# gcorso/DiffDock

Hardware: AMD Instinct MI355X
Metric: poses/sec (20 steps x 40 samples, DiffDock-L score model) (higher is better)
Workload: dtype f32

## Files before the change

diffdock_amd/csrc/api.cpp:

```cpp
#include <cstdlib>
#include <cstring>

#include "model.h"

using namespace ddmi;

struct ddmi_model { Model m; };

static thread_local std::string g_err;

template <class F> static int guard(F&& f) {
  try { f(); return DDMI_OK; }
  catch (const Error& e) { g_err = e.what(); return e.code; }
  catch (const std::exception& e) { g_err = e.what(); return DDMI_ERR_ARG; }
}

extern "C" {

const char* ddmi_last_error(void) { return g_err.c_str(); }

int ddmi_create(const ddmi_config* cfg, int device, ddmi_model** out) {
  return guard([&] {
    DDMI_REQUIRE(cfg && out, DDMI_ERR_ARG, "null argument");
    DDMI_REQUIRE(cfg->struct_size == sizeof(ddmi_config), DDMI_ERR_ARG,
                 "ddmi_config.struct_size != sizeof(ddmi_config) of this library: the caller was built against another include/ddmi.h");
    DDMI_CHECK_HIP(hipSetDevice(device));
    auto* h = new ddmi_model();
    h->m.cfg = *cfg;
    h->m.device = device;
    try { build_weight_spec(h->m); } catch (...) { delete h; throw; }
    {
      const ddmi_exec_options& x = h->m.cfg.exec;
      auto in = [&](int v, int hi, const char* name) {
        if (v < 0 || v > hi) { delete h; throw Error(DDMI_ERR_ARG, std::string("ddmi_config.exec.") + name + ": out of range"); }
      };
      if (h->m.cfg.edge_product < 0 || h->m.cfg.edge_product > 1) { delete h; throw Error(DDMI_ERR_ARG, "ddmi_config.edge_product: 0 (f32) or 1 (bf16x4)"); }
      in(x.streams, 1, "streams"); in(x.dense_rows, 2, "dense_rows"); in(x.shared_tiles, 2, "shared_tiles");
      in(x.packed_granules, 1, "packed_granules"); in(x.merged_granule, 1, "merged_granule"); in(x.pre_reduce, 1, "pre_reduce");
      in(x.hidden_mm, 1, "hidden_mm"); in(x.fc1_batch, 1, "fc1_batch"); in(x.tile_split, 8, "tile_split");
      in(x.tile_split_small, 8, "tile_split_small"); in(x.hidden_grid, 1 << 20, "hidden_grid"); in(x.tp_apply, 3, "tp_apply");
      in(x.tile_per_pose, 1, "tile_per_pose"); in(x.layer_overlap, 2, "layer_overlap");
      in(x.grouped, 2, "grouped"); in(x.grouped_split, 8, "grouped_split"); in(x.vn_build, 1, "vn_build"); in(x.node_update, 3, "node_update"); in(x.tile_split_last, 8, "tile_split_last"); in(x.tile_split_rule, 2, "tile_split_rule"); in(x.group_order, 3, "group_order"); in(x.list_caps, 1, "list_caps"); in(x.time_terms, 1, "time_terms");
      h->m.two_streams = x.streams == 0;
      h->m.fused_dense = x.dense_rows == 0 ? 1 : x.dense_rows == 1 ? 0 : 2;
      h->m.fused_shared = x.shared_tiles == 0 ? 1 : x.shared_tiles == 1 ? 0 : 2;
      h->m.fused_pack = x.packed_granules == 0;
      h->m.fused_tri = x.merged_granule == 0;
      h->m.fused_prered = x.pre_reduce == 0;
      h->m.fused_mm = x.hidden_mm == 0;
      h->m.fc1_batch = x.fc1_batch == 0;
      h->m.fused_ysplit = x.tile_split;
      h->m.fused_ysplit_small = x.tile_split_small;
      h->m.eh_grid = x.hidden_grid > 0 ? x.hidden_grid : 2048;
      h->m.tp_form = x.tp_apply == 0 ? -1 : x.tp_apply - 1;
      h->m.tile_per_pose = x.tile_per_pose != 0;
      h->m.layer_overlap = x.layer_overlap;
      h->m.grouped = x.grouped;
      h->m.grouped_split = x.grouped_split;
      h->m.vn_merge = x.vn_build == 0;
      h->m.node_update = x.node_update >= 1;
      h->m.node_update_wpn = x.node_update == 2 ? 1 : x.node_update == 3 ? 4 : 0;
      h->m.fused_ysplit_last = x.tile_split_last;
      h->m.ys_rounds = x.tile_split_rule != 1;
      h->m.ys_rounds_small = x.tile_split_rule == 2;
      h->m.group_order = x.group_order;
      h->m.tight_caps = x.list_caps == 1;
      h->m.time_terms_fused = x.time_terms == 1;
      {
        int cus = 0;
        if (hipDeviceGetAttribute(&cus, hipDeviceAttributeMultiprocessorCount, device) == hipSuccess && cus >= 16) h->m.n_cus = cus;
      }
    }
    DDMI_CHECK_HIP(hipStreamCreateWithFlags(&h->m.side_stream, hipStreamNonBlocking));
    DDMI_CHECK_HIP(hipEventCreate(&h->m.ev_fork));
    DDMI_CHECK_HIP(hipEventCreate(&h->m.ev_join));
    DDMI_CHECK_HIP(hipEventCreate(&h->m.ev_cross));
    DDMI_CHECK_HIP(hipEventCreate(&h->m.ev_terms));
    *out = h;
  });
}

void ddmi_destroy(ddmi_model* h) {
  if (!h) return;
  Model& m = h->m;
  if (m.side_stream) { (void)hipStreamSynchronize(m.side_stream); (void)hipStreamDestroy(m.side_stream); }
  for (hipEvent_t e : {m.ev_fork, m.ev_join, m.ev_cross, m.ev_terms}) if (e) (void)hipEventDestroy(e);
  for (hipEvent_t e : m.ev_pipe) (void)hipEventDestroy(e);
  delete h;
}

int ddmi_num_weights(ddmi_model* h) { return h ? (int)h->m.spec.size() : DDMI_ERR_ARG; }

int ddmi_weight_spec(ddmi_model* h, int i, const char** key, int64_t shape[4], int* ndim) {
  return guard([&] {
    DDMI_REQUIRE(h && i >= 0 && i < (int)h->m.spec.size(), DDMI_ERR_ARG, "bad index");
    *key = h->m.spec[i].first.c_str();
    *ndim = (int)h->m.spec[i].second.size();
    for (int d = 0; d < *ndim; ++d) shape[d] = h->m.spec[i].second[d];
  });
}

int ddmi_set_weight(ddmi_model* h, const char* key, const float* data, const int64_t* shape, int ndim) {
  return guard([&] {
    DDMI_REQUIRE(h && key && shape && ndim >= 1 && ndim <= 4, DDMI_ERR_ARG, "bad argument");
    int64_t numel = 1;
    for (int d = 0; d < ndim; ++d) numel *= shape[d];
    DDMI_REQUIRE(data || numel == 0, DDMI_ERR_ARG, "null data");
    Model& m = h->m;
    bool known = false;
    for (auto& kv : m.spec) if (kv.first == key) {
      known = true;
      DDMI_REQUIRE((int)kv.second.size() == ndim && std::equal(shape, shape + ndim, kv.second.begin()), DDMI_ERR_KEY,
                   std::string("shape mismatch for ") + key);
    }
    DDMI_REQUIRE(known, DDMI_ERR_KEY, std::string("unexpected state_dict key: ") + key);
    HostTensor t;
    t.shape.assign(shape, shape + ndim);
    if (numel) t.data.assign(data, data + numel);
    m.host_w[key] = std::move(t);
    m.committed = false;
  });
}

int ddmi_commit_weights(ddmi_model* h) {
  return guard([&] { DDMI_REQUIRE(h, DDMI_ERR_ARG, "null model"); DDMI_CHECK_HIP(hipSetDevice(h->m.device)); commit_weights(h->m); });
}

int ddmi_set_table(ddmi_model* h, int kind, const double* data, int64_t n) {
  return guard([&] {
    DDMI_REQUIRE(h && data && n > 1 && (kind == 0 || kind == 1), DDMI_ERR_ARG, "bad table");
    DDMI_CHECK_HIP(hipSetDevice(h->m.device));
    std::vector<float> f(data, data + n);
    float* p = h->m.tpool.upload(f);
    if (kind == 0) { h->m.so3_table = p; h->m.so3_n = (int)n; }
    else { h->m.torus_table = p; h->m.torus_n = (int)n; }
  });
}

int ddmi_set_time_frequencies(ddmi_model* h, const float* freq, int64_t n) {
  return guard([&] {
    DDMI_REQUIRE(h && freq && n == h->m.cfg.sigma_embed_dim / 2, DDMI_ERR_ARG, "need sigma_embed_dim/2 frequencies");
    DDMI_REQUIRE(!h->m.committed, DDMI_ERR_STATE, "set frequencies before ddmi_commit_weights");
    h->m.time_freq_host.assign(freq, freq + n);
  });
}

int ddmi_set_complex(ddmi_model* h, const ddmi_complex* c, ddmi_stream s) {
  return guard([&] {
    DDMI_REQUIRE(h && c, DDMI_ERR_ARG, "null argument");
    DDMI_CHECK_HIP(hipSetDevice(h->m.device));
// ... 145 lines not shown
```

diffdock_amd/csrc/complex.cpp:

```cpp
#include <algorithm>
#include <cmath>
#include <numeric>
#include <string>
#include <cstdlib>

#include "model.h"

namespace ddmi {

struct Model::Cx {
  int B = 0, nL = 0, nR = 0, N = 0, Eb = 0, Err = 0, nT = 0;
  int maxNl = 0, maxNr = 0, Ell_cap = 0, Elr_cap = 0, tor_cap = 32, Et = 0, lig_cap = 33;
  bool uniform = false; int Nl_one = 0, R_one = 0;
  std::vector<int> lig_ptr_h, rec_ptr_h;
  int *lig_batch, *rec_batch, *lig_ptr, *rec_ptr, *lig_x;
  int *bond_src, *bond_dst, *bond_grank, *bond_trank, *bg, *bt; float* bond_attr;
  int *tor_u, *tor_v, *tor_batch, *tor_eu, *tor_ev, *rot_u, *rot_v; unsigned char* mask_rotate = nullptr;
  float* rec_pos; int *rr_src, *rr_dst, *rr_batch; float *rr_dist, *rr_nvec, *rr_ew, *rec_edge_base;
  int *rr_goff, *rr_tgt, *rr_tslot, *rr_arow, *rr_toff, *rr_tlist, *rr_gnode;
  int *keep, *cnt_g2, *cnt_t2, *goff2, *toff2, *tslot_tmp, *tgt2, *tslot2, *arow2;
  ReduceGroup *rg_all_crop, *rg_rr_crop;
  float* rec_node_enc;
  float* rec_node_base; int rec_base_dim = 0;
  float *temb, *hidB, *rec_sig, *ligsig, *ll_gvec, *cross_gvec, *center_gvec, *tr_sig, *rot_sig, *cutoff, *rr_rowbias;
  float *ac_in = nullptr, *ac_h0 = nullptr, *ac_h1 = nullptr, *ac_out = nullptr;
  float* rr_sig_old = nullptr;
  float* embsum;
  std::vector<float*> X;
  int *adjrank, *cnt_g, *cnt_t, *goff_ll, *toff_ll, *ll_tgt, *ll_tslot, *ll_featidx, *ll_batch;
  float *ll_dist, *ll_nvec, *ll_ew, *ll_ea;
  int *pairrank, *cnt_l, *cnt_r, *offs_l, *offs_r, *g1_tgt, *g1_tslot, *g3_tgt, *g3_tslot, *pbatch;
  float *pdist, *pnvec, *pew, *cross_ea;
  float *HE, *P, *Q; float* msg[4];
  const float* x_last = nullptr;
  float *HE_b, *P_b, *Q_b, *rowbias_b;
  float *Pg[9] = {}, *Qg[9] = {}, *rbg[9] = {};
  struct VnSet { int vcap = 0; int *cnt = nullptr, *voff = nullptr, *node = nullptr, *e0 = nullptr, *ne = nullptr;
                 float* rows = nullptr;
                 int* tile_hdr = nullptr; unsigned char* live = nullptr;
                 int* nvn_pad = nullptr;
                 const int *built_goff = nullptr, *built_tgt = nullptr, *built_tslot = nullptr, *built_arow = nullptr;
                 const float *built_nvec = nullptr, *built_ew = nullptr; float built_sgn = 0.f; int built_tbase = -1; long epoch = -1; };
  bool prered = false;
  VnSet vn[9];
  int nA = 0, maxNa = 0, Eaa = 0, Ear = 0, Ela_cap = 0;
  int *atom_batch = nullptr, *atom_ptr = nullptr, *atom_x = nullptr;
  float* atom_pos = nullptr;
  struct StaticEdges { int E = 0; int *goff = nullptr, *toff = nullptr, *arow = nullptr, *tgt = nullptr, *tslot = nullptr; };
  StaticEdges se_aa, se_ar, se_ra;
  int *aa_batch = nullptr, *ar_batch = nullptr;
  float *aa_dist = nullptr, *aa_nvec = nullptr, *aa_ew = nullptr, *atom_edge_base = nullptr;
  float *ar_dist = nullptr, *ar_nvec = nullptr, *ar_edge_base = nullptr, *atom_node_base = nullptr;
  int *la_pairrank = nullptr, *la_cnt_l = nullptr, *la_cnt_a = nullptr, *la_offs_l = nullptr, *la_offs_a = nullptr;
  int *la1_tgt = nullptr, *la1_tslot = nullptr, *la3_tgt = nullptr, *la3_tslot = nullptr, *la_pbatch = nullptr;
  float *la_dist = nullptr, *la_nvec = nullptr, *la_ew = nullptr, *la_ea = nullptr, *la_gvec = nullptr;
  float* msg_aa[9] = {};
  ReduceGroup *rg_aa_all = nullptr, *rg_aa_lig = nullptr;
  long epoch = 0;
  float *Hb = nullptr, *Hb_b = nullptr;
  std::vector<float*> rb_l;
  float* Hbg[9] = {};
  float *HD[2] = {nullptr, nullptr}, *HD_b[2] = {nullptr, nullptr};
  ReduceGroup *rg_all, *rg_lig, *rg_ll, *rg_rr;
  float *c_dist, *c_nvec, *c_ea, *c_attr, *c_hid, *c_W, *c_sh, *c_out, *gp;
  int* c_xrow;
  int *t_cnt, *t_atom; float *t_dist, *t_nvec, *t_ew, *t_bond_nvec, *t_ea, *t_attr, *t_hid, *t_W, *t_sh, *t_out, *t_feat;
  float *s_tr, *s_rot, *s_tor, *s_t = nullptr; long long* s_ids = nullptr;
  long long* s_ids_host = nullptr; hipEvent_t s_ids_ev = nullptr;
  ~Cx() { if (s_ids_host) (void)hipHostFree(s_ids_host); if (s_ids_ev) (void)hipEventDestroy(s_ids_ev); }
};

static hipEvent_t get_event(Model& m) {
  if (!m.free_events.empty()) { hipEvent_t e = m.free_events.back(); m.free_events.pop_back(); return e; }
  hipEvent_t e;
  DDMI_CHECK_HIP(hipEventCreate(&e));
  return e;
}
PhaseTimer::PhaseTimer(Model& model, const char* name, hipStream_t stream) : m(model), s(stream) {
  if (!m.timing) return;
  for (size_t i = 0; i < m.phases.size(); ++i) if (m.phases[i].name == name) idx = (int)i;
  if (idx < 0) { m.phases.push_back({name, 0.0, 0}); idx = (int)m.phases.size() - 1; }
  a = get_event(m); b = get_event(m);
  (void)hipEventRecord(a, s);
}
PhaseTimer::~PhaseTimer() {
  if (idx < 0) return;
  (void)hipEventRecord(b, s);
  m.pending.push_back({idx, a, b});
}
void resolve_timings(Model& m) {
  for (auto& p : m.pending) {
    (void)hipEventSynchronize(p.b);
    float ms = 0.f;
    if (hipEventElapsedTime(&ms, p.a, p.b) == hipSuccess) { m.phases[p.phase].ms += ms; m.phases[p.phase].launches++; }
    m.free_events.push_back(p.a); m.free_events.push_back(p.b);
  }
  m.pending.clear();
}

namespace {

typedef Model::Cx Cx;

template <class T> T* dalloc(Model& m, const char* name, std::vector<int64_t> shape, bool zero = false) {
  size_t n = 1;
  for (auto d : shape) n *= (size_t)std::max<int64_t>(d, 0);
  T* p = m.cpool.alloc<T>(n ? n : 1);
  if (zero) DDMI_CHECK_HIP(hipMemset(p, 0, (n ? n : 1) * sizeof(T)));
  if (name) m.debug[name] = DebugEntry{p, shape, !std::is_same<T, float>::value};
  return p;
}
template <class T> T* dup(Model& m, const char* name, const std::vector<T>& v) {
  T* p = m.cpool.upload(v);
  if (name) m.debug[name] = DebugEntry{p, {(int64_t)v.size()}, !std::is_same<T, float>::value};
  return p;
}

void gemm(const float* A, int lda, const float* W, int ldw, const float* bias, float* C, int ldc, int M, int N, int K,
          int act, hipStream_t s, const int* m_dev = nullptr, const float* rowbias = nullptr, const int* ridx = nullptr,
          int ldrb = 0) {
  GemmArgs g;
  g.A = A; g.lda = lda; g.W = W; g.ldw = ldw; g.bias = bias; g.C = C; g.ldc = ldc; g.M = M; g.N = N; g.K = K; g.act = act;
  g.m_dev = m_dev; g.rowbias = rowbias; g.ridx = ridx; g.ldrb = ldrb;
  launch_gemm(g, s);
}

struct RunGroup {
  int gbase, gcount, tbase, tcount;
  const int *goff, *tgt, *tslot, *arow;
  const float* ea; int ea_rows; const int* ea_rows_dev;
  const float* sig; const int* sig_idx;
  const float *nvec, *ew; float sgn;
  float* msg;
  int vn = -1;
  bool load = false;
  bool swap_pq = false;
  const float* rb_ready = nullptr;
  bool static_topo = false;
};

static long tiles_of(const RunGroup& q) {
  const long gn = std::max(1, q.gcount);
  return std::max(1L, gn * (((long)q.ea_rows / gn + 31) / 32) / 16);
}

static bool vn_fresh(const Cx& c, const RunGroup& g) {
  const Cx::VnSet& vs = c.vn[g.vn];
  return vs.built_goff == g.goff && (vs.epoch == c.epoch || (g.static_topo && vs.epoch >= 0)) && vs.built_tgt == g.tgt && vs.built_tslot == g.tslot &&
         vs.built_arow == g.arow && vs.built_nvec == g.nvec && vs.built_ew == g.ew && vs.built_sgn == g.sgn && vs.built_tbase == g.tbase;
}
static void vn_mark_built(Cx& c, const RunGroup& g) {
  Cx::VnSet& vs = c.vn[g.vn];
  vs.built_goff = g.goff; vs.epoch = c.epoch; vs.built_tgt = g.tgt; vs.built_tslot = g.tslot; vs.built_arow = g.arow;
  vs.built_nvec = g.nvec; vs.built_ew = g.ew; vs.built_sgn = g.sgn; vs.built_tbase = g.tbase;
}
static VnRowsArgs vn_rows_args(const Model& m, const RunGroup& g) {
  const Cx::VnSet& vs = m.cx->vn[g.vn];
  VnRowsArgs vr{};
  vr.arow = g.arow; vr.nvec = g.nvec; vr.ew = g.ew; vr.tslot = g.tslot; vr.sgn = g.sgn; vr.sh_lmax = m.cfg.sh_lmax;
  vr.tgt = g.tgt; vr.tbase = g.tbase;
  vr.vcap = vs.vcap; vr.rows = vs.rows; vr.vn_ne = vs.ne;
  return vr;
}
static const char vn_type[9] = {'R', 'R', 'L', 'L', 'A', 'A', 'A', 'L', 'R'};
static void ensure_vn_all(Model& m, const std::vector<RunGroup>& groups, hipStream_t gs) {
  Cx& c = *m.cx;
  VnListsArgs LA;
  VnRowsArgs rows[VN_GROUPS_MAX];
  const RunGroup* prered_g = nullptr;
  for (auto& g : groups) {
    if (vn_fresh(c, g) || g.gcount <= 0) continue;
    DDMI_REQUIRE(LA.n < VN_GROUPS_MAX, DDMI_ERR_CAPACITY, "more edge groups than virtual-node list slots");
    Cx::VnSet& vs = c.vn[g.vn];
    VnListArgs& a = LA.g[LA.n];
    a = VnListArgs{g.goff, g.gcount, vs.voff, vs.node, vs.e0, nullptr, nullptr, 0, nullptr};
    if (vs.nvn_pad) {
      const bool lig = vn_type[g.vn] == 'L', atom = vn_type[g.vn] == 'A';
      a.node_batch = lig ? c.lig_batch : atom ? c.atom_batch : c.rec_batch;
      a.graph_ptr = lig ? c.lig_ptr : atom ? c.atom_ptr : c.rec_ptr;
      a.n_graphs = c.B; a.nvn_pad = vs.nvn_pad;
    }
    rows[LA.n] = vn_rows_args(m, g);
    if (g.vn == 0 && c.prered) {
      prered_g = &g;
      if (m.cfg.sh_lmax <= 1) { rows[LA.n].tile_hdr = vs.tile_hdr; rows[LA.n].live = vs.live; }
    }
    ++LA.n;
    vn_mark_built(c, g);
  }
  if (LA.n == 0) return;
  PhaseTimer t(m, "vn_build", gs);
  launch_vn_build_all(LA, rows, m.cfg.sh_lmax, gs);
  if (prered_g && m.cfg.sh_lmax > 1) {
    Cx::VnSet& vs = c.vn[0];
    launch_vn_tiles(vs.nvn_pad ? vs.nvn_pad : vs.voff + prered_g->gcount, vs.vcap, vs.rows, vs.ne, vs.tile_hdr, vs.live, gs);
  }
}
static void ensure_vn(Model& m, const RunGroup& g, hipStream_t gs) {
  Cx& c = *m.cx;
  Cx::VnSet& vs = c.vn[g.vn];
  if (vn_fresh(c, g)) return;
  PhaseTimer t(m, "vn_build", gs);
  const VnRowsArgs vr = vn_rows_args(m, g);
  VnPoseTiles pp{};
  if (vs.nvn_pad) {
    const bool lig = vn_type[g.vn] == 'L', atom = vn_type[g.vn] == 'A';
    pp.node_batch = lig ? c.lig_batch : atom ? c.atom_batch : c.rec_batch;
    pp.graph_ptr = lig ? c.lig_ptr : atom ? c.atom_ptr : c.rec_ptr;
    pp.n_graphs = c.B; pp.nvn_pad = vs.nvn_pad;
  }
  launch_vn_build(g.goff, g.gcount, vs.cnt, vs.voff, vs.node, vs.e0, vr, gs, vs.nvn_pad ? &pp : nullptr);
  if (g.vn == 0 && c.prered) launch_vn_tiles(vs.nvn_pad ? vs.nvn_pad : vs.voff + g.gcount, vs.vcap, vs.rows, vs.ne, vs.tile_hdr, vs.live, gs);
  vn_mark_built(c, g);
}

struct GroupRoute { bool bf, dense_rows; };
static GroupRoute group_route(const Model& m, const ConvW& L, const RunGroup& g) {
  GroupRoute r;
  r.bf = m.cfg.edge_product == 1 && !L.fgran_generic && L.maxd <= 3 && m.cfg.sh_lmax <= 1;
  r.dense_rows = m.fused_dense == 2 || (m.fused_dense == 1 && (long)g.ea_rows >= 20L * std::max(1, g.gcount));
  return r;
}

static EdgeHiddenArgs hidden_args(Model& m, const ConvW& L, const RunGroup& g, int wg, const float* P, const float* Q, const float* rb,
                                  float* Hb, const GroupRoute& rt) {
  Cx& c = *m.cx;
  Cx::VnSet& vs = c.vn[g.vn];
  EdgeHiddenArgs h{};
  h.nvn = vs.nvn_pad ? vs.nvn_pad : vs.voff + g.gcount;
  h.vcap = vs.vcap; h.vn_node = vs.node; h.vn_e0 = vs.e0; h.goff = g.goff; h.arow = g.arow; h.tgt = g.tgt;
  h.tbase = g.tbase; h.ea = g.ea; h.ns = m.ns; h.W1 = L.W1p[wg]; h.ldw = L.n_edge; h.P = P; h.Q = Q; h.rowbias = rb; h.ridx = g.sig_idx;
  h.H = L.H; h.NG8 = L.HKq / 8; h.Hb = Hb; h.bf = rt.bf ? 1 : 0;
  h.zero_fill = (!L.fgran_generic && rt.dense_rows) ? 1 : 0;
  if (m.cfg.sh_lmax <= 1) { h.vrows = vs.rows; h.vn_ne = vs.ne; }
  h.grid = m.eh_grid;
  return h;
}

static FusedConvArgs fused_args(Model& m, const ConvW& L, const RunGroup& g, size_t gi, int wg, const float* Xin, const float* Hb,
                                const GroupRoute& rt, bool small_layer, int ys_force) {
  Cx& c = *m.cx;
  Cx::VnSet& vs = c.vn[g.vn];
  FusedConvArgs f{};
  f.nvn = vs.nvn_pad ? vs.nvn_pad : vs.voff + g.gcount;
  f.vcap = vs.vcap; f.vn_node = vs.node; f.vrows = vs.rows; f.vn_ne = vs.ne;
  f.X = Xin; f.gbase = g.gbase; f.wpack = L.wpack[wg]; f.KS = L.KS; f.HK = L.HK; f.Hb = Hb; f.NG8 = L.HKq / 8;
  f.sh_lmax = m.cfg.sh_lmax; f.gran = L.fgran; f.cgt = L.cgt;
  f.max_nb = L.max_nb; f.maxd = L.maxd; f.msg = g.msg; f.generic = L.fgran_generic ? 1 : 0;
  f.dense = rt.dense_rows ? 1 : 0;
  f.bf = rt.bf ? 1 : 0;
  f.tile_hdr = (g.vn == 0 && c.prered) ? vs.tile_hdr : nullptr;
  f.shared = (rt.dense_rows && (m.fused_shared == 2 || (m.fused_shared == 1 && g.load && (long)g.ea_rows >= 48L * std::max(1, g.gcount)))) ? 1 : 0;
  f.prof_slot = (int)gi;
  int ys_req = ys_force > 0 ? ys_force : m.fused_ysplit;
  if (ys_req <= 0) {
    auto round_model = [&](long T) {
      int pick = 1;
      double best = 1e30;
      for (int y = 1; y <= std::min(8, L.n_fgran); ++y) {
        const double rounds = std::ceil((double)T * y / (double)m.n_cus);
        const double cost = rounds * ((double)((L.n_fgran + y - 1) / y) + 0.2);
        if (cost < best - 1e-9) { best = cost; pick = y; }
      }
      return pick;
    };
    if (small_layer && m.ys_rounds_small && tiles_of(g) >= 32) ys_req = round_model(tiles_of(g));
    else if (small_layer) ys_req = (int)std::min(8L, std::max(1L, 768 / tiles_of(g)));
    else if (m.ys_rounds && tiles_of(g) >= m.n_cus) {
      ys_req = round_model(tiles_of(g));
    }
    else ys_req = (int)std::min(6L, std::max(1L, 768 / std::max(1L, ((long)g.gcount + g.ea_rows / 32) / 16)));
    const int ys_small = m.fused_ysplit_small;
    if (ys_small > 0 && !small_layer && tiles_of(g) < 256) ys_req = ys_small;
  }
  ys_req = std::max(ys_req, (L.n_fgran + 19) / 20);
  const int ys = std::max(1, std::min(std::min(ys_req, 8), L.n_fgran));
  f.ysplit = ys;
  f.gsplit[0] = 0;
  for (int y = 1; y < ys; ++y) {
    int b = L.n_fgran * y / ys;
    while (b < L.n_fgran && b > 0 && L.fgran_unit[b] == L.fgran_unit[b - 1]) ++b;
    f.gsplit[y] = std::max(b, f.gsplit[y - 1]);
  }
  f.gsplit[ys] = L.n_fgran;
  f.n_units = 0;
  for (int gq = 0; gq < L.n_fgran && f.n_units < 48; ++gq)
    if (gq == 0 || L.fgran_unit[gq] != L.fgran_unit[gq - 1]) f.ustart[f.n_units++] = (short)gq;
  for (int y = 0; y < ys; ++y) {
    f.ufirst[y] = 0; f.ucount[y] = 0;
    for (int u = 0; u < f.n_units; ++u)
      if (f.ustart[u] >= f.gsplit[y] && f.ustart[u] < f.gsplit[y + 1]) { if (f.ucount[y] == 0) f.ufirst[y] = (short)u; ++f.ucount[y]; }
  }
// ... 72 lines not shown
    launch_conv_fused(f, gs);
  }
}

static bool grouped_ok(const Model& m, const ConvW& L, const std::vector<RunGroup>& groups) {
  const Cx& c = *m.cx;
  if (!c.Hbg[0] || groups.size() < 2 || groups.size() > 9 || !c.Pg[0]) return false;
  if (L.TL != 2 || !m.fused_mm || m.ns % 16 != 0 || m.ns > 64 || L.fgran_generic || L.maxd > 3 || m.cfg.sh_lmax > 1 || L.n_fgran <= 0) return false;
  if (m.cfg.edge_product != 0) return false;
  if (m.timing && m.timing_level >= 2) return false;
  for (size_t gi = 0; gi < groups.size(); ++gi)
    if (!L.W1p[std::min<int>((int)gi, L.G - 1)] || groups[gi].vn < 0) return false;
  return true;
}
static void run_groups_grouped(Model& m, const ConvW& L, const std::vector<RunGroup>& groups, const float* Xin, hipStream_t s, bool pq_ready) {
  Cx& c = *m.cx;
  const int ns = m.ns, H = L.H;
  if (!pq_ready) {
    PhaseTimer t(m, "conv_fc1_gemms", s);
    GemmBatch gb;
    auto add = [&](const float* A, int lda, const float* W, const float* bias, float* C, int M) {
      if (gb.n == GEMM_BATCH_MAX) { launch_gemm_batch(gb, s); gb.n = 0; }
      GemmArgs& x = gb.g[gb.n++];
      x = GemmArgs{};
      x.A = A; x.lda = lda; x.W = W; x.ldw = L.n_edge; x.bias = bias; x.C = C; x.ldc = H; x.M = M; x.N = H; x.K = ns;
    };
    for (size_t gi = 0; gi < groups.size(); ++gi) {
      const RunGroup& g = groups[gi];
      const int wg = std::min<int>((int)gi, L.G - 1);
      const float* W1p = L.W1p[wg];
      if (g.sig && !g.rb_ready) add(g.sig, ns, W1p, nullptr, c.rbg[gi], c.B);
      add(Xin + (size_t)g.tbase * XS, XS, W1p + (g.swap_pq ? 2 : 1) * ns, nullptr, c.Pg[gi], g.tcount);
      add(Xin + (size_t)g.gbase * XS, XS, W1p + (g.swap_pq ? 1 : 2) * ns, L.b1p[wg], c.Qg[gi], g.gcount);
    }
    launch_gemm_batch(gb, s);
  }
  ensure_vn_all(m, groups, s);
  long tiles = 0;
  for (auto& g : groups) tiles += tiles_of(g);
  int ys = m.grouped_split;
  if (ys <= 0) ys = (int)std::min(8L, std::max(1L, (long)m.grouped_target / std::max(1L, tiles)));
  std::vector<size_t> order(groups.size());
  std::iota(order.begin(), order.end(), 0);
  std::stable_sort(order.begin(), order.end(), [&](size_t a, size_t b) {
    const GroupRoute ra = group_route(m, L, groups[a]), rb_ = group_route(m, L, groups[b]);
    if (ra.dense_rows != rb_.dense_rows) return ra.dense_rows;
    return tiles_of(groups[a]) > tiles_of(groups[b]);
  });
  for (size_t o0 = 0; o0 < order.size(); o0 += FC_GROUPS_MAX) {
    const size_t n = std::min<size_t>(FC_GROUPS_MAX, order.size() - o0);
    EdgeHiddenGroupedArgs HG;
    FusedGroupedArgs FG;
    HG.n = FG.n = (int)n;
    for (size_t k = 0; k < n; ++k) {
      const size_t gi = order[o0 + k];
      const RunGroup& g = groups[gi];
      const int wg = std::min<int>((int)gi, L.G - 1);
      const GroupRoute rt = group_route(m, L, g);
      HG.g[k] = hidden_args(m, L, g, wg, c.Pg[gi], c.Qg[gi], g.sig ? (g.rb_ready ? g.rb_ready : c.rbg[gi]) : nullptr, c.Hbg[g.vn], rt);
      HG.g[k].grid = std::max(64, (int)((long)m.eh_grid * tiles_of(g) / std::max(1L, tiles)));
      FG.g[k] = fused_args(m, L, g, gi, wg, Xin, c.Hbg[g.vn], rt, false, ys);
    }
    {
      PhaseTimer t(m, "k_edge_hidden", s);
      launch_edge_hidden_mm_grouped(HG, s);
    }
    PhaseTimer t(m, "k_conv_fused", s);
    launch_conv_grouped(FG, s);
  }
}

void run_conv(Model& m, const ConvW& L, const std::vector<RunGroup>& groups, const ReduceGroup* rg_dev, int n_rg,
              const float* Xin, float* Xout, int nbase, int ncount, hipStream_t s, int pq_mode = 0, const ConvW* Lnext = nullptr,
              const std::vector<RunGroup>* gnext = nullptr) {
  Cx& c = *m.cx;
  const int ns = m.ns, H = L.H;
  auto node_update = [&]() {
    if (!Lnext) {
      PhaseTimer t(m, "k_reduce_bn", s);
      launch_reduce_bn(rg_dev, n_rg, nbase, ncount, L.D_in, L.D_out, L.has_bn ? L.bn_mean : nullptr,
                       L.has_bn ? L.bn_scale : nullptr, L.has_bn ? L.bn_bias : nullptr, L.residual ? 1 : 0, Xin, Xout, XS, s);
      return;
    }
    PhaseTimer t(m, "k_reduce_bn", s);
    NodeUpdateArgs a{};
    a.groups = rg_dev; a.n_groups = n_rg; a.nbase = nbase; a.ncount = ncount; a.D_in = L.D_in; a.D_out = L.D_out;
    a.bn_mean = L.has_bn ? L.bn_mean : nullptr; a.bn_scale = L.has_bn ? L.bn_scale : nullptr; a.bn_bias = L.has_bn ? L.bn_bias : nullptr;
    a.residual = L.residual ? 1 : 0; a.X_in = Xin; a.X_out = Xout;
    a.ns = ns; a.H = Lnext->H; a.ldw = Lnext->n_edge; a.wpn = m.node_update_wpn;
    for (size_t gi = 0; gi < gnext->size(); ++gi) {
      const RunGroup& g = (*gnext)[gi];
      const int wg = std::min<int>((int)gi, Lnext->G - 1);
      const float* W1p = Lnext->W1p[wg];
      DDMI_REQUIRE(a.n_terms + 2 <= NU_TERMS_MAX, DDMI_ERR_CAPACITY, "k_node_update: more first-Linear terms than slots");
      a.term[a.n_terms++] = NodeTerm{W1p + (g.swap_pq ? 2 : 1) * ns, nullptr, c.Pg[gi], g.tbase, g.tcount};
      a.term[a.n_terms++] = NodeTerm{W1p + (g.swap_pq ? 1 : 2) * ns, Lnext->b1p[wg], c.Qg[gi], g.gbase, g.gcount};
    }
    launch_node_update(a, s);
  };
  bool forked = false;
  if (m.two_streams && m.side_stream && groups.size() > 1) {
    for (auto& g : groups) forked = forked || (g.gbase == 0 && g.gcount == c.nL && c.nR > 0);
    bool any_main = false;
    for (auto& g : groups) any_main = any_main || !(g.gbase == 0 && g.gcount == c.nL);
    forked = forked && any_main;
  }
  long biggest = 1;
  for (auto& q : groups) biggest = std::max(biggest, tiles_of(q));
  const bool small_layer = biggest < 256;
  if (m.grouped == 2 && grouped_ok(m, L, groups)) {
    run_groups_grouped(m, L, groups, Xin, s, pq_mode == 2);
    node_update();
    return;
  }
  bool mm_all = L.TL == 2 && (pq_mode != 0 || (m.fc1_batch && small_layer)) && m.fused_mm && ns % 16 == 0 && ns <= 64 && groups.size() <= 9 && c.Pg[0];
  for (size_t gi = 0; gi < groups.size(); ++gi) mm_all = mm_all && L.W1p[std::min<int>((int)gi, L.G - 1)];
  DDMI_REQUIRE(pq_mode == 0 || mm_all, DDMI_ERR_STATE, "fused node-update route on a layer without batched first-Linear terms");
  if (mm_all && pq_mode != 2) {
    PhaseTimer t(m, "conv_fc1_gemms", s);
    GemmBatch gb;
    auto add = [&](const float* A, int lda, const float* W, const float* bias, float* C, int M) {
      if (gb.n == GEMM_BATCH_MAX) { launch_gemm_batch(gb, s); gb.n = 0; }
      GemmArgs& x = gb.g[gb.n++];
      x = GemmArgs{};
      x.A = A; x.lda = lda; x.W = W; x.ldw = L.n_edge; x.bias = bias; x.C = C; x.ldc = H; x.M = M; x.N = H; x.K = ns;
    };
    for (size_t gi = 0; gi < groups.size(); ++gi) {
      const RunGroup& g = groups[gi];
      const int wg = std::min<int>((int)gi, L.G - 1);
      const float* W1p = L.W1p[wg];
      if (g.sig && !g.rb_ready) add(g.sig, ns, W1p, nullptr, c.rbg[gi], c.B);
      add(Xin + (size_t)g.tbase * XS, XS, W1p + (g.swap_pq ? 2 : 1) * ns, nullptr, c.Pg[gi], g.tcount);
      add(Xin + (size_t)g.gbase * XS, XS, W1p + (g.swap_pq ? 1 : 2) * ns, L.b1p[wg], c.Qg[gi], g.gcount);
    }
    launch_gemm_batch(gb, s);
  }
  if (m.vn_merge) ensure_vn_all(m, groups, s);
  if (forked) {
    DDMI_CHECK_HIP(hipEventRecord(m.ev_fork, s));
    DDMI_CHECK_HIP(hipStreamWaitEvent(m.side_stream, m.ev_fork, 0));
  }
  std::vector<size_t> issue;
  for (int pass = 0; pass < 2; ++pass) {
    std::vector<size_t> part;
    for (size_t gi = 0; gi < groups.size(); ++gi) {
      const bool side_g = forked && groups[gi].gbase == 0 && groups[gi].gcount == c.nL;
      if (side_g == (pass == 1)) part.push_back(gi);
    }
    if (forked && ((m.group_order >> (pass == 1 ? 0 : 1)) & 1)) std::reverse(part.begin(), part.end());
    issue.insert(issue.end(), part.begin(), part.end());
  }
  if (!forked || m.group_order == 0) { issue.clear(); for (size_t gi = 0; gi < groups.size(); ++gi) issue.push_back(gi); }
  for (size_t ii = 0; ii < issue.size(); ++ii) {
    const size_t gi = issue[ii];
    const RunGroup& g = groups[gi];
    const bool side = forked && g.gbase == 0 && g.gcount == c.nL;
    int ys_last = 0;
    if (m.fused_ysplit_last > 0 && !small_layer) {
      bool last_on_stream = true;
      for (size_t jj = ii + 1; jj < issue.size(); ++jj) {
        const size_t gj = issue[jj];
        const bool side_j = forked && groups[gj].gbase == 0 && groups[gj].gcount == c.nL;
        if (side_j == side) last_on_stream = false;
      }
      if (last_on_stream && tiles_of(g) >= 256) ys_last = m.fused_ysplit_last;
    }
// ... 119 lines not shown
    const int nl = c.lig_ptr_h[b + 1] - c.lig_ptr_h[b], nr = c.rec_ptr_h[b + 1] - c.rec_ptr_h[b];
    DDMI_REQUIRE(nl > 0 && nr > 0, DDMI_ERR_ARG, "graph without ligand or receptor nodes");
    c.maxNl = std::max(c.maxNl, nl); c.maxNr = std::max(c.maxNr, nr);
    c.Elr_cap += nl * nr;
    if (nl != c.lig_ptr_h[1]) c.uniform = false;
    for (int i = c.lig_ptr_h[b]; i < c.lig_ptr_h[b + 1]; ++i) lig_batch[i] = b;
    for (int i = c.rec_ptr_h[b]; i < c.rec_ptr_h[b + 1]; ++i) rec_batch[i] = b;
  }
  c.Ell_cap = c.Eb + c.lig_cap * c.nL;
  std::vector<int> atom_ptr_h, atom_batch, aa_tl, aa_gl, ar_atom, ar_rec, aa_batch_h, ar_batch_h;
  struct HostEdges { std::vector<int> goff, toff, arow, tgt, tslot; };
  auto build_static = [&](const std::vector<int>& tl, const std::vector<int>& gl, int n_t, int n_g, int tgt_base) {
    HostEdges h;
    const int E = (int)tl.size();
    h.goff.assign(n_g + 1, 0); h.toff.assign(n_t + 1, 0);
    for (int k = 0; k < E; ++k) {
      DDMI_REQUIRE(tl[k] >= 0 && tl[k] < n_t && gl[k] >= 0 && gl[k] < n_g, DDMI_ERR_ARG, "atom edge index out of range");
      h.goff[gl[k] + 1]++; h.toff[tl[k] + 1]++;
    }
    for (int i = 0; i < n_g; ++i) h.goff[i + 1] += h.goff[i];
    for (int i = 0; i < n_t; ++i) h.toff[i + 1] += h.toff[i];
    h.arow.resize(E); h.tgt.resize(E); h.tslot.resize(E);
    std::vector<int> cur(h.goff.begin(), h.goff.end() - 1), tcur(h.toff.begin(), h.toff.end() - 1);
    for (int k = 0; k < E; ++k) h.arow[cur[gl[k]]++] = k;
    for (int e = 0; e < E; ++e) { const int k = h.arow[e]; h.tgt[e] = tgt_base + tl[k]; h.tslot[e] = tcur[tl[k]]++; }
    return h;
  };
  HostEdges h_aa, h_ar, h_ra;
  if (cfg.all_atoms) {
    atom_ptr_h.assign(cc.atom_ptr, cc.atom_ptr + c.B + 1);
    DDMI_REQUIRE(atom_ptr_h[0] == 0 && atom_ptr_h[c.B] == c.nA, DDMI_ERR_ARG, "atom_ptr does not span the atom array");
    atom_batch.resize(c.nA);
    for (int b = 0; b < c.B; ++b) {
      const int na = atom_ptr_h[b + 1] - atom_ptr_h[b], nl = c.lig_ptr_h[b + 1] - c.lig_ptr_h[b];
      c.maxNa = std::max(c.maxNa, na);
      c.Ela_cap += nl * na;
      for (int i = atom_ptr_h[b]; i < atom_ptr_h[b + 1]; ++i) atom_batch[i] = b;
    }
    std::vector<int> aa_index(2 * (size_t)c.Eaa), ar_index(2 * (size_t)c.Ear);
    DDMI_CHECK_HIP(hipMemcpy(aa_index.data(), cc.atom_edge_index, aa_index.size() * 4, hipMemcpyDeviceToHost));
    DDMI_CHECK_HIP(hipMemcpy(ar_index.data(), cc.atom_rec_edge_index, ar_index.size() * 4, hipMemcpyDeviceToHost));
    aa_tl.assign(aa_index.begin(), aa_index.begin() + c.Eaa); aa_gl.assign(aa_index.begin() + c.Eaa, aa_index.end());
    ar_atom.assign(ar_index.begin(), ar_index.begin() + c.Ear); ar_rec.assign(ar_index.begin() + c.Ear, ar_index.end());
    h_aa = build_static(aa_tl, aa_gl, c.nA, c.nA, c.nL + c.nR);
    h_ar = build_static(ar_atom, ar_rec, c.nA, c.nR, c.nL + c.nR);
    h_ra = build_static(ar_rec, ar_atom, c.nR, c.nA, c.nL);
    aa_batch_h.resize(c.Eaa); ar_batch_h.resize(c.Ear);
    for (int k = 0; k < c.Eaa; ++k) aa_batch_h[k] = atom_batch[aa_tl[k]];
    for (int k = 0; k < c.Ear; ++k) ar_batch_h[k] = atom_batch[ar_atom[k]];
  }
  std::vector<int> bsrc(c.Eb), bdst(c.Eb), bgr(c.Eb), btr(c.Eb), bg(c.nL, 0), bt(c.nL, 0);
  for (int k = 0; k < c.Eb; ++k) {
    bsrc[k] = bond_index[k]; bdst[k] = bond_index[c.Eb + k];
    DDMI_REQUIRE(bsrc[k] >= 0 && bsrc[k] < c.nL && bdst[k] >= 0 && bdst[k] < c.nL, DDMI_ERR_ARG, "bond index out of range");
    bgr[k] = bg[bdst[k]]++;
    btr[k] = bt[bsrc[k]]++;
  }
  std::vector<int> tor_u, tor_v, tor_b;
  for (int k = 0; k < c.Eb && !cfg.no_torsion; ++k)
    if (edge_mask[k]) { tor_u.push_back(bsrc[k]); tor_v.push_back(bdst[k]); tor_b.push_back(lig_batch[bsrc[k]]); }
  DDMI_REQUIRE((int)tor_u.size() == c.nT, DDMI_ERR_ARG, "n_tor does not equal edge_mask.sum()");
  c.Et = c.nT * c.tor_cap;
  std::vector<int> tor_eu(c.Et), tor_ev(c.Et);
  for (int t = 0; t < c.nT; ++t)
    for (int r = 0; r < c.tor_cap; ++r) { tor_eu[t * c.tor_cap + r] = tor_u[t]; tor_ev[t * c.tor_cap + r] = tor_v[t]; }
  std::vector<int> rr_src(c.Err), rr_dst(c.Err), rr_batch(c.Err), goff(c.nR + 1, 0), toff(c.nR + 1, 0);
  for (int k = 0; k < c.Err; ++k) {
    rr_src[k] = rr_index[k]; rr_dst[k] = rr_index[c.Err + k];
    DDMI_REQUIRE(rr_src[k] >= 0 && rr_src[k] < c.nR && rr_dst[k] >= 0 && rr_dst[k] < c.nR, DDMI_ERR_ARG, "receptor edge out of range");
    rr_batch[k] = rec_batch[rr_src[k]];
    goff[rr_dst[k] + 1]++; toff[rr_src[k] + 1]++;
  }
  for (int i = 0; i < c.nR; ++i) { goff[i + 1] += goff[i]; toff[i + 1] += toff[i]; }
  std::vector<int> rr_arow(c.Err), rr_tgt(c.Err), rr_tslot(c.Err), cur(goff.begin(), goff.end() - 1), tcur(toff.begin(), toff.end() - 1);
  for (int k = 0; k < c.Err; ++k) rr_arow[cur[rr_dst[k]]++] = k;
  std::vector<int> rr_tlist(c.Err), rr_gnode(c.Err);
  for (int e = 0; e < c.Err; ++e) {
    const int k = rr_arow[e];
    rr_tgt[e] = c.nL + rr_src[k];
    rr_tslot[e] = tcur[rr_src[k]]++;
    rr_tlist[rr_tslot[e]] = e;
    rr_gnode[e] = rr_dst[k];
  }
  if (cfg.all_atoms) {
    c.atom_batch = dup(m, "atom_batch", atom_batch); c.atom_ptr = dup(m, nullptr, atom_ptr_h);
    c.atom_x = dalloc<int>(m, nullptr, {c.nA * 4});
    DDMI_CHECK_HIP(hipMemcpy(c.atom_x, cc.atom_x, (size_t)c.nA * 4 * 4, hipMemcpyDeviceToDevice));
    c.atom_pos = dalloc<float>(m, nullptr, {c.nA * 3});
    DDMI_CHECK_HIP(hipMemcpy(c.atom_pos, cc.atom_pos, (size_t)c.nA * 12, hipMemcpyDeviceToDevice));
    auto up_edges = [&](const HostEdges& h, const char* name) {
      Cx::StaticEdges e;
      e.E = (int)h.arow.size();
      e.goff = dup(m, name, h.goff); e.toff = dup(m, nullptr, h.toff); e.arow = dup(m, nullptr, h.arow);
      e.tgt = dup(m, nullptr, h.tgt); e.tslot = dup(m, nullptr, h.tslot);
      return e;
    };
    c.se_aa = up_edges(h_aa, "aa_goff"); c.se_ar = up_edges(h_ar, "ar_goff"); c.se_ra = up_edges(h_ra, "ra_goff");
    c.aa_batch = dup(m, nullptr, aa_batch_h); c.ar_batch = dup(m, nullptr, ar_batch_h);
    int* aa_src = dup(m, nullptr, aa_tl); int* aa_dst = dup(m, nullptr, aa_gl);
    int* ar_src = dup(m, nullptr, ar_atom); int* ar_dst = dup(m, nullptr, ar_rec);
    c.aa_dist = dalloc<float>(m, nullptr, {c.Eaa}); c.aa_nvec = dalloc<float>(m, nullptr, {c.Eaa, 3});
    c.aa_ew = cfg.smooth_edges ? dalloc<float>(m, nullptr, {c.Eaa}) : nullptr;
    c.ar_dist = dalloc<float>(m, nullptr, {c.Ear}); c.ar_nvec = dalloc<float>(m, nullptr, {c.Ear, 3});
    c.atom_edge_base = dalloc<float>(m, nullptr, {c.Eaa, ns}); c.ar_edge_base = dalloc<float>(m, nullptr, {c.Ear, ns});
    c.atom_node_base = dalloc<float>(m, "atom_node_base", {c.nA, XS}, true);
    launch_rec_edge_geom(c.atom_pos, aa_src, aa_dst, c.Eaa, cfg.smooth_edges ? cfg.lig_max_radius : 0.f, c.aa_dist, c.aa_nvec,
                         c.aa_ew, s);
    float* rp = dalloc<float>(m, nullptr, {c.nR * 3});
    DDMI_CHECK_HIP(hipMemcpy(rp, cc.rec_pos, (size_t)c.nR * 12, hipMemcpyDeviceToDevice));
    launch_rec_edge_geom(c.atom_pos, ar_src, ar_dst, c.Ear, 0.f, c.ar_dist, c.ar_nvec, nullptr, s, rp);
  }
  c.lig_batch = dup(m, "lig_batch", lig_batch); c.rec_batch = dup(m, "rec_batch", rec_batch);
  c.lig_ptr = dup(m, nullptr, c.lig_ptr_h); c.rec_ptr = dup(m, nullptr, c.rec_ptr_h);
  c.lig_x = dalloc<int>(m, nullptr, {c.nL * 16});
  DDMI_CHECK_HIP(hipMemcpy(c.lig_x, cc.lig_x, (size_t)c.nL * 16 * 4, hipMemcpyDeviceToDevice));
  c.bond_src = dup(m, nullptr, bsrc); c.bond_dst = dup(m, nullptr, bdst); c.bond_grank = dup(m, nullptr, bgr);
  c.bond_trank = dup(m, nullptr, btr); c.bg = dup(m, nullptr, bg); c.bt = dup(m, nullptr, bt);
  c.bond_attr = dalloc<float>(m, nullptr, {c.Eb * m.nf});
  if (c.Eb) DDMI_CHECK_HIP(hipMemcpy(c.bond_attr, cc.bond_attr, (size_t)c.Eb * m.nf * 4, hipMemcpyDeviceToDevice));
  c.tor_u = dup(m, "tor_u", tor_u); c.tor_v = dup(m, "tor_v", tor_v); c.tor_batch = dup(m, nullptr, tor_b);
  c.tor_eu = dup(m, nullptr, tor_eu); c.tor_ev = dup(m, nullptr, tor_ev);
  if (c.uniform && c.nT % c.B == 0) {
    c.Nl_one = c.nL / c.B; c.R_one = c.nT / c.B;
    std::vector<int> ru(tor_u.begin(), tor_u.begin() + c.R_one), rv(tor_v.begin(), tor_v.begin() + c.R_one);
    c.rot_u = dup(m, nullptr, ru); c.rot_v = dup(m, nullptr, rv);
    if (cc.mask_rotate && c.R_one > 0) {
      c.mask_rotate = dalloc<unsigned char>(m, nullptr, {c.R_one * c.Nl_one});
      DDMI_CHECK_HIP(hipMemcpy(c.mask_rotate, cc.mask_rotate, (size_t)c.R_one * c.Nl_one, hipMemcpyDeviceToDevice));
    }
  }
  c.rec_pos = dalloc<float>(m, nullptr, {c.nR * 3});
  DDMI_CHECK_HIP(hipMemcpy(c.rec_pos, cc.rec_pos, (size_t)c.nR * 12, hipMemcpyDeviceToDevice));
  c.rr_src = dup(m, nullptr, rr_src); c.rr_dst = dup(m, nullptr, rr_dst); c.rr_batch = dup(m, nullptr, rr_batch);
  c.rr_goff = dup(m, "rr_goff", goff); c.rr_toff = dup(m, "rr_toff", toff); c.rr_arow = dup(m, nullptr, rr_arow);
  c.rr_tgt = dup(m, nullptr, rr_tgt); c.rr_tslot = dup(m, nullptr, rr_tslot);
  c.rr_tlist = dup(m, nullptr, rr_tlist); c.rr_gnode = dup(m, nullptr, rr_gnode);
  c.keep = dalloc<int>(m, "crop_keep", {c.nR}); c.cnt_g2 = dalloc<int>(m, nullptr, {c.nR}); c.cnt_t2 = dalloc<int>(m, nullptr, {c.nR});
  c.goff2 = dalloc<int>(m, "rr_goff_crop", {c.nR + 1}); c.toff2 = dalloc<int>(m, nullptr, {c.nR + 1});
  c.tslot_tmp = dalloc<int>(m, nullptr, {c.Err}); c.tgt2 = dalloc<int>(m, nullptr, {c.Err});
  c.tslot2 = dalloc<int>(m, nullptr, {c.Err}); c.arow2 = dalloc<int>(m, nullptr, {c.Err});
  const int B = c.B, nL = c.nL, nR = c.nR, N = c.N;
  c.rr_dist = dalloc<float>(m, nullptr, {c.Err}); c.rr_nvec = dalloc<float>(m, nullptr, {c.Err, 3});
  c.rr_ew = cfg.smooth_edges ? dalloc<float>(m, nullptr, {c.Err}) : nullptr;
  c.rec_edge_base = dalloc<float>(m, "rec_edge_base", {c.Err, ns});
  c.rec_node_base = dalloc<float>(m, "rec_node_base", {nR, XS}, true);
  c.temb = dalloc<float>(m, "temb", {B, sd}); c.hidB = dalloc<float>(m, nullptr, {B, std::max(ns, H)});
  c.rec_sig = dalloc<float>(m, "rec_sig", {B, ns}); c.ligsig = dalloc<float>(m, nullptr, {B, ns});
  c.ll_gvec = dalloc<float>(m, nullptr, {B, ns}); c.cross_gvec = dalloc<float>(m, nullptr, {B, ns});
  c.center_gvec = dalloc<float>(m, nullptr, {B, ns}); c.tr_sig = dalloc<float>(m, nullptr, {B, ns});
  c.rr_sig_old = dalloc<float>(m, nullptr, {B, ns});
  if (cfg.atom_confidence && cfg.confidence_mode) {
    c.ac_in = dalloc<float>(m, nullptr, {nL, 2 * ns}); c.ac_h0 = dalloc<float>(m, nullptr, {nL, ns});
    c.ac_h1 = dalloc<float>(m, nullptr, {nL, ns}); c.ac_out = dalloc<float>(m, nullptr, {nL, cfg.atom_num_confidence_outputs + ns});
  }
  c.rot_sig = dalloc<float>(m, nullptr, {B, ns}); c.cutoff = dalloc<float>(m, "cross_cutoff", {B});
  c.rr_rowbias = dalloc<float>(m, nullptr, {B, H});
  c.embsum = dalloc<float>(m, nullptr, {nL, ns});
  const int n_layers = cfg.old_model ? cfg.num_conv_layers + 2 : (int)m.conv_layers.size(), K = (int)m.lig_emb_layers.size();
  for (int l = 0; l <= n_layers + K; ++l) {
    static const char* names[] = {"x0", "x1", "x2", "x3", "x4", "x5", "x6", "x7", "x8", "x9", "x10", "x11", "x12"};
    c.X.push_back(dalloc<float>(m, l < 13 ? names[l] : nullptr, {N, XS}, true));
  }
  c.adjrank = dalloc<int>(m, nullptr, {nL, c.maxNl}); c.cnt_g = dalloc<int>(m, nullptr, {nL}); c.cnt_t = dalloc<int>(m, nullptr, {nL});
  c.goff_ll = dalloc<int>(m, "goff_ll", {nL + 1}); c.toff_ll = dalloc<int>(m, "toff_ll", {nL + 1});
  c.ll_tgt = dalloc<int>(m, "ll_tgt", {c.Ell_cap}); c.ll_tslot = dalloc<int>(m, nullptr, {c.Ell_cap});
  c.ll_featidx = dalloc<int>(m, nullptr, {c.Ell_cap}); c.ll_batch = dalloc<int>(m, nullptr, {c.Ell_cap});
  c.ll_dist = dalloc<float>(m, "ll_dist", {c.Ell_cap}); c.ll_nvec = dalloc<float>(m, nullptr, {c.Ell_cap, 3});
  c.ll_ew = cfg.smooth_edges ? dalloc<float>(m, nullptr, {c.Ell_cap}) : nullptr;
  c.ll_ea = dalloc<float>(m, "ll_ea", {c.Ell_cap, ns});
  c.pairrank = dalloc<int>(m, nullptr, {nL, c.maxNr}); c.cnt_l = dalloc<int>(m, nullptr, {nL}); c.cnt_r = dalloc<int>(m, nullptr, {nR});
  c.offs_l = dalloc<int>(m, "offs_l", {nL + 1}); c.offs_r = dalloc<int>(m, "offs_r", {nR + 1});
  c.g1_tgt = dalloc<int>(m, nullptr, {c.Elr_cap}); c.g1_tslot = dalloc<int>(m, nullptr, {c.Elr_cap});
  c.g3_tgt = dalloc<int>(m, nullptr, {c.Elr_cap}); c.g3_tslot = dalloc<int>(m, nullptr, {c.Elr_cap});
  c.pbatch = dalloc<int>(m, nullptr, {c.Elr_cap}); c.pdist = dalloc<float>(m, "cross_dist", {c.Elr_cap});
  c.pnvec = dalloc<float>(m, nullptr, {c.Elr_cap, 3}); c.pew = cfg.smooth_edges ? dalloc<float>(m, nullptr, {c.Elr_cap}) : nullptr;
  c.cross_ea = dalloc<float>(m, "cross_ea", {c.Elr_cap, ns});
  const int max_rows = std::max(std::max(std::max(c.Ell_cap, c.Elr_cap), std::max(c.Err, c.Eaa)), std::max(c.Ear, c.Ela_cap));
  c.HE = dalloc<float>(m, nullptr, {max_rows, H}); c.P = dalloc<float>(m, nullptr, {N, H}); c.Q = dalloc<float>(m, nullptr, {N, H});
  c.HE_b = dalloc<float>(m, nullptr, {std::max(std::max(c.Ell_cap, c.Elr_cap), c.Ela_cap), H}); c.P_b = dalloc<float>(m, nullptr, {N, H});
  c.Q_b = dalloc<float>(m, nullptr, {N, H}); c.rowbias_b = dalloc<float>(m, nullptr, {B, H});
  if (cfg.tp_weights_layers > 2) {
    for (int i = 0; i < 2; ++i) {
      c.HD[i] = dalloc<float>(m, nullptr, {max_rows, H});
      c.HD_b[i] = dalloc<float>(m, nullptr, {std::max(std::max(c.Ell_cap, c.Elr_cap), c.Ela_cap), H});
    }
  }
  for (int i = 0; i < (cfg.all_atoms ? 9 : 4); ++i) {
    c.Pg[i] = dalloc<float>(m, nullptr, {N, H}); c.Qg[i] = dalloc<float>(m, nullptr, {N, H}); c.rbg[i] = dalloc<float>(m, nullptr, {B, H});
  }
  for (size_t l = 0; l < m.conv_layers.size(); ++l) c.rb_l.push_back(dalloc<float>(m, nullptr, {B, H}));
  std::vector<const ConvW*> all_layers;
  for (auto* fam : {&m.conv_layers, &m.lig_emb_layers, &m.rec_emb_layers, &m.old_lig, &m.old_rec, &m.old_l2r, &m.old_r2l})
    for (auto& L : *fam) all_layers.push_back(&L);
  {
    int HKq = 0;
    for (auto* L : all_layers) HKq = std::max(HKq, L->HKq);
    const int ecap_v[9] = {c.Elr_cap, c.Err, c.Ell_cap, c.Elr_cap, c.Ela_cap, c.Ear, c.Eaa, c.Ela_cap, c.Ear};
    const int gn_v[9] = {nR, nR, nL, nL, c.nA, c.nA, c.nA, nL, nR};
    const bool lig_v[9] = {false, false, true, true, false, false, false, true, false};
    const char* names[9] = {"vn_off_cross", "vn_off_rr", "vn_off_ll", "vn_off_rl", "vn_off_la", "vn_off_ra", "vn_off_aa",
                            "vn_off_al", "vn_off_ar"};
    long tight[9];
    for (int i = 0; i < 9; ++i) tight[i] = -1;
    auto vn_of = [](long deg) { return (deg + 31) / 32; };
    auto exact = [&](const std::vector<int>& off) { long n = 0; for (size_t d = 0; d + 1 < off.size(); ++d) n += vn_of(off[d + 1] - off[d]); return n; };
    tight[0] = tight[3] = 0;
    for (int b = 0; b < B; ++b) {
      const long nl = c.lig_ptr_h[b + 1] - c.lig_ptr_h[b], nr = c.rec_ptr_h[b + 1] - c.rec_ptr_h[b];
      tight[0] += nr * vn_of(nl);
      tight[3] += nl * vn_of(nr);
    }
    tight[1] = exact(goff);
    tight[2] = 0;
    for (int d = 0; d < nL; ++d) tight[2] += vn_of((long)c.lig_cap + bg[d]);
    if (cfg.all_atoms) {
      tight[4] = tight[7] = 0;
      for (int b = 0; b < B; ++b) {
        const long nl = c.lig_ptr_h[b + 1] - c.lig_ptr_h[b], na = atom_ptr_h[b + 1] - atom_ptr_h[b];
        tight[4] += na * vn_of(nl);
        tight[7] += nl * vn_of(na);
      }
      tight[5] = exact(h_ra.goff); tight[6] = exact(h_aa.goff); tight[8] = exact(h_ar.goff);
    }
    int vmax = 0, vmax_b = 0;
    for (int i = 0; i < (cfg.all_atoms ? 9 : 4); ++i) {
      Cx::VnSet& vs = c.vn[i];
      vs.vcap = gn_v[i] + ecap_v[i] / 32 + 2;
      if (m.tight_caps && tight[i] >= 0) vs.vcap = (int)std::min<long>(vs.vcap, tight[i] + 2);
      if (m.tile_per_pose) {
        vs.vcap += 16 * B;
        vs.nvn_pad = dalloc<int>(m, i == 0 ? "vn_count_cross" : nullptr, {1}, true);
      }
      vs.cnt = dalloc<int>(m, nullptr, {gn_v[i] + 1}); vs.voff = dalloc<int>(m, names[i], {gn_v[i] + 1});
      vs.node = dalloc<int>(m, nullptr, {vs.vcap}); vs.e0 = dalloc<int>(m, nullptr, {vs.vcap});
      const int shd = (cfg.sh_lmax + 1) * (cfg.sh_lmax + 1);
      vs.ne = dalloc<int>(m, i == 0 ? "vn_ne_cross" : nullptr, {round_up(vs.vcap, 16)});
      vs.rows = dalloc<float>(m, nullptr, {round_up(vs.vcap, 16), 32, shd == 4 ? 8 : shd + 3});
      if (i == 0) {
        c.prered = m.fused_prered && shd == 4 && !cfg.old_model && !m.conv_layers.empty() && m.fused_shared != 2;
        for (auto& L : m.conv_layers) c.prered = c.prered && !L.fgran_generic && L.maxd <= 3 && L.n_fgran > 0;
        if (c.prered) {
          vs.tile_hdr = dalloc<int>(m, "prered_tile_hdr", {round_up(vs.vcap, 16) / 16, FC_TILE_HDR}, true);
          vs.live = dalloc<unsigned char>(m, nullptr, {ecap_v[0]}, true);
        }
      }
      vmax = std::max(vmax, vs.vcap);
      if (lig_v[i]) vmax_b = std::max(vmax_b, vs.vcap);
    }
    c.Hb = HKq > 0 ? dalloc<float>(m, nullptr, {round_up(vmax, 16), 32, round_up(HKq, 16)}) : nullptr;
    if (m.grouped == 2 && HKq > 0)
      for (int i = 0; i < (cfg.all_atoms ? 9 : 4); ++i) c.Hbg[i] = dalloc<float>(m, nullptr, {round_up(c.vn[i].vcap, 16), 32, round_up(HKq, 16)});
    c.Hb_b = HKq > 0 ? dalloc<float>(m, nullptr, {round_up(vmax_b, 16), 32, round_up(HKq, 16)}) : nullptr;
  }
  const int ecap[4] = {c.Ell_cap, c.Elr_cap, c.Err, c.Elr_cap};
  for (int g = 0; g < 4; ++g) c.msg[g] = dalloc<float>(m, nullptr, {ecap[g], XS});
  {
    std::vector<ReduceGroup> rg = {{c.toff_ll, c.msg[0], 0, nL}, {c.offs_l, c.msg[1], 0, nL},
                                   {c.rr_toff, c.msg[2], nL, nR}, {c.offs_r, c.msg[3], nL, nR}};
    rg[1].live = c.prered ? c.vn[0].live : nullptr;
    c.rg_all = m.cpool.upload(rg);
    std::vector<ReduceGroup> rl(rg.begin(), rg.begin() + 2);
    c.rg_lig = m.cpool.upload(rl);
    std::vector<ReduceGroup> r0(rg.begin(), rg.begin() + 1);
    c.rg_ll = m.cpool.upload(r0);
    std::vector<ReduceGroup> r2 = {{c.rr_toff, c.msg[2], 0, nR}};
    c.rg_rr = m.cpool.upload(r2);
    std::vector<ReduceGroup> rc = rg;
    rc[2].toff = c.toff2;
    c.rg_all_crop = m.cpool.upload(rc);
    std::vector<ReduceGroup> r2c = {{c.toff2, c.msg[2], nL, nR}};
    c.rg_rr_crop = m.cpool.upload(r2c);
    if (cfg.all_atoms) {
      const int nA = c.nA;
      c.la_pairrank = dalloc<int>(m, nullptr, {nL, c.maxNa}); c.la_cnt_l = dalloc<int>(m, nullptr, {nL});
      c.la_cnt_a = dalloc<int>(m, nullptr, {nA}); c.la_offs_l = dalloc<int>(m, "offs_la_l", {nL + 1});
      c.la_offs_a = dalloc<int>(m, "offs_la_a", {nA + 1});
      c.la1_tgt = dalloc<int>(m, nullptr, {c.Ela_cap}); c.la1_tslot = dalloc<int>(m, nullptr, {c.Ela_cap});
      c.la3_tgt = dalloc<int>(m, nullptr, {c.Ela_cap}); c.la3_tslot = dalloc<int>(m, nullptr, {c.Ela_cap});
      c.la_pbatch = dalloc<int>(m, nullptr, {c.Ela_cap}); c.la_dist = dalloc<float>(m, nullptr, {c.Ela_cap});
      c.la_nvec = dalloc<float>(m, nullptr, {c.Ela_cap, 3});
      c.la_ew = cfg.smooth_edges ? dalloc<float>(m, nullptr, {c.Ela_cap}) : nullptr;
      c.la_ea = dalloc<float>(m, nullptr, {c.Ela_cap, ns}); c.la_gvec = dalloc<float>(m, nullptr, {B, ns});
      const int ecap9[9] = {c.Ell_cap, c.Elr_cap, c.Ela_cap, c.Err, c.Elr_cap, c.Ear, c.Eaa, c.Ela_cap, c.Ear};
      for (int g = 0; g < 9; ++g) c.msg_aa[g] = (g == 0 || g == 1 || g == 3 || g == 4) ? c.msg[g == 0 ? 0 : g == 1 ? 1 : g == 3 ? 2 : 3]
                                                                                          : dalloc<float>(m, nullptr, {ecap9[g], XS});
      std::vector<ReduceGroup> r9 = {{c.toff_ll, c.msg_aa[0], 0, nL}, {c.offs_l, c.msg_aa[1], 0, nL}, {c.la_offs_l, c.msg_aa[2], 0, nL},
                                     {c.rr_toff, c.msg_aa[3], nL, nR}, {c.offs_r, c.msg_aa[4], nL, nR}, {c.se_ra.toff, c.msg_aa[5], nL, nR},
                                     {c.se_aa.toff, c.msg_aa[6], nL + nR, nA}, {c.la_offs_a, c.msg_aa[7], nL + nR, nA},
                                     {c.se_ar.toff, c.msg_aa[8], nL + nR, nA}};
      r9[1].live = c.prered ? c.vn[0].live : nullptr;
      c.rg_aa_all = m.cpool.upload(r9);
      std::vector<ReduceGroup> r3(r9.begin(), r9.begin() + 3);
      c.rg_aa_lig = m.cpool.upload(r3);
    }
  }
  const ConvW& F = m.final_conv;
  c.c_dist = dalloc<float>(m, nullptr, {nL}); c.c_nvec = dalloc<float>(m, nullptr, {nL, 3});
  c.c_ea = dalloc<float>(m, nullptr, {nL, ns}); c.c_attr = dalloc<float>(m, nullptr, {nL, F.n_edge});
  c.c_hid = dalloc<float>(m, nullptr, {nL, F.H}); c.c_W = dalloc<float>(m, nullptr, {nL, F.Wn});
  c.c_sh = dalloc<float>(m, nullptr, {nL, F.sh_dim}); c.c_out = dalloc<float>(m, nullptr, {nL, F.D_out});
  c.gp = dalloc<float>(m, "global_pred", {B, F.D_out});
  {
    std::vector<int> xr(nL);
    std::iota(xr.begin(), xr.end(), 0);
    c.c_xrow = m.cpool.upload(xr);
  }
  if (c.nT > 0) {
    const ConvW& T = m.tor_conv;
    c.t_cnt = dalloc<int>(m, "tor_cnt", {c.nT}); c.t_atom = dalloc<int>(m, nullptr, {c.Et});
    c.t_dist = dalloc<float>(m, nullptr, {c.Et}); c.t_nvec = dalloc<float>(m, nullptr, {c.Et, 3});
    c.t_ew = cfg.smooth_edges ? dalloc<float>(m, nullptr, {c.Et}) : nullptr;
    c.t_bond_nvec = dalloc<float>(m, nullptr, {c.nT, 3}); c.t_ea = dalloc<float>(m, nullptr, {c.Et, ns});
    c.t_attr = dalloc<float>(m, nullptr, {c.Et, T.n_edge}); c.t_hid = dalloc<float>(m, nullptr, {c.Et, T.H});
    c.t_W = dalloc<float>(m, nullptr, {c.Et, T.Wn}); c.t_sh = dalloc<float>(m, nullptr, {c.Et, T.sh_dim});
    c.t_out = dalloc<float>(m, nullptr, {c.Et, T.D_out}); c.t_feat = dalloc<float>(m, "tor_feat", {c.nT, T.D_out});
  }
  c.s_tr = dalloc<float>(m, nullptr, {B, 3}); c.s_rot = dalloc<float>(m, nullptr, {B, 3});
  c.s_tor = dalloc<float>(m, nullptr, {std::max(c.nT, 1)});
  c.s_t = nullptr; c.s_ids = nullptr;

  launch_rec_edge_geom(c.rec_pos, c.rr_src, c.rr_dst, c.Err, cfg.smooth_edges ? cfg.rec_max_radius : 0.f, c.rr_dist, c.rr_nvec,
                       c.rr_ew, s);
  if (!cfg.old_model)
    launch_edge_mlp(mlp_args(m.rec_edge, ns, c.Err, nullptr, c.rr_dist, m.off_rec, m.D, m.coeff_rec, 0, m.rec_edge.b0, nullptr,
                             c.rec_edge_base), s);
  if (cfg.old_model) {
    std::vector<int> ident(nR);
    std::iota(ident.begin(), ident.end(), 0);
    int* rid = m.cpool.upload(ident);
    float* cat = dalloc<float>(m, nullptr, {nR, ns + m.lm});
    launch_concat_rec_input(cc.rec_x, 1 + m.lm, m.rec_emb, ns, m.lm, nR, cat, s);
    if (m.lm > 0) {
      float* emb1 = dalloc<float>(m, nullptr, {nR, ns});
      gemm(cat + ns, ns + m.lm, m.old_rec_lin.W0, sd, m.old_rec_lin.b0, emb1, ns, nR, ns, sd, 0, s, nullptr, cat, rid, ns + m.lm);
      gemm(emb1, ns, m.old_lm_W, ns + m.lm, m.old_lm_b, c.rec_node_base, XS, nR, ns, ns, 0, s);
      gemm(cat + ns + sd, ns + m.lm, m.old_lm_W + ns, ns + m.lm, nullptr, c.rec_node_base, XS, nR, ns, m.lm - sd, 0, s, nullptr,
           c.rec_node_base, rid, XS);
    } else {
      launch_add_rowvec(c.rec_node_base, XS, cat, ns, nullptr, 0, nullptr, nR, ns, 0, s);
    }
  } else if (m.lm > 0) {
    float* cat = dalloc<float>(m, nullptr, {nR, ns + m.lm});
    launch_concat_rec_input(cc.rec_x, 1 + m.lm, m.rec_emb, ns, m.lm, nR, cat, s);
    gemm(cat, ns + m.lm, m.rec_enc_W, ns + m.lm, m.rec_enc_b, c.rec_node_base, XS, nR, ns, ns + m.lm, 0, s);
  } else {
    float* cat = dalloc<float>(m, nullptr, {nR, ns});
    launch_concat_rec_input(cc.rec_x, 1, m.rec_emb, ns, 0, nR, cat, s);
    launch_add_rowvec(c.rec_node_base, XS, cat, ns, nullptr, 0, nullptr, nR, ns, 0, s);
  }
  c.rec_base_dim = ns;
  if (cfg.all_atoms) {
    float* emb = dalloc<float>(m, nullptr, {c.nA, ns});
    launch_lig_node_embed(c.atom_x, c.nA, m.atom_emb, m.atom_emb_off, 4, ns, emb, s);
    launch_add_rowvec(c.atom_node_base, XS, emb, ns, nullptr, 0, nullptr, c.nA, ns, 0, s);
    launch_edge_mlp(mlp_args(m.atom_edge, ns, c.Eaa, nullptr, c.aa_dist, m.off_lig, m.D, m.coeff_lig, 0, m.atom_edge.b0, nullptr,
                             c.atom_edge_base), s);
    launch_edge_mlp(mlp_args(m.ar_edge, ns, c.Ear, nullptr, c.ar_dist, m.off_rec, m.D, m.coeff_rec, 0, m.ar_edge.b0, nullptr,
                             c.ar_edge_base), s);
  }
  c.rec_node_enc = nullptr;
  if (!m.rec_emb_layers.empty() && cfg.all_atoms) {
    const int aB = nL + nR, nA = c.nA;
    float* ea = dalloc<float>(m, nullptr, {N, XS}, true);
    float* eb = dalloc<float>(m, nullptr, {N, XS}, true);
    DDMI_CHECK_HIP(hipMemcpyAsync(ea + (size_t)nL * XS, c.rec_node_base, (size_t)nR * XS * 4, hipMemcpyDeviceToDevice, s));
    DDMI_CHECK_HIP(hipMemcpyAsync(ea + (size_t)aB * XS, c.atom_node_base, (size_t)nA * XS * 4, hipMemcpyDeviceToDevice, s));
    RunGroup e_rr{nL, nR, nL, nR, c.rr_goff, c.rr_tgt, c.rr_tslot, c.rr_arow, c.rec_edge_base, c.Err, nullptr, nullptr, nullptr,
                  c.rr_nvec, c.rr_ew, 1.f, c.msg_aa[3]};
    RunGroup e_ar{nL, nR, aB, nA, c.se_ar.goff, c.se_ar.tgt, c.se_ar.tslot, c.se_ar.arow, c.ar_edge_base, c.Ear, nullptr, nullptr,
                  nullptr, c.ar_nvec, nullptr, 1.f, c.msg_aa[8]};
    RunGroup e_aa{aB, nA, aB, nA, c.se_aa.goff, c.se_aa.tgt, c.se_aa.tslot, c.se_aa.arow, c.atom_edge_base, c.Eaa, nullptr, nullptr,
                  nullptr, c.aa_nvec, c.aa_ew, 1.f, c.msg_aa[6]};
    RunGroup e_ra{aB, nA, nL, nR, c.se_ra.goff, c.se_ra.tgt, c.se_ra.tslot, c.se_ra.arow, c.ar_edge_base, c.Ear, nullptr, nullptr,
                  nullptr, c.ar_nvec, nullptr, 1.f, c.msg_aa[5]};
    e_rr.vn = 1; e_ar.vn = 8; e_aa.vn = 6; e_ra.vn = 5;
    std::vector<ReduceGroup> re = {{c.rr_toff, c.msg_aa[3], nL, nR}, {c.se_ar.toff, c.msg_aa[8], aB, nA},
                                   {c.se_aa.toff, c.msg_aa[6], aB, nA}, {c.se_ra.toff, c.msg_aa[5], nL, nR}};
    ReduceGroup* rg_emb = m.cpool.upload(re);
    float *xin = ea, *xout = eb;
    for (size_t i = 0; i < m.rec_emb_layers.size(); ++i) {
      run_conv(m, m.rec_emb_layers[i], {e_rr, e_ar, e_aa, e_ra}, rg_emb, 4, xin, xout, nL, nR + nA, s);
      std::swap(xin, xout);
      c.rec_base_dim = m.rec_emb_layers[i].D_out;
    }
    DDMI_CHECK_HIP(hipMemcpyAsync(c.rec_node_base, xin + (size_t)nL * XS, (size_t)nR * XS * 4, hipMemcpyDeviceToDevice, s));
    DDMI_CHECK_HIP(hipMemcpyAsync(c.atom_node_base, xin + (size_t)aB * XS, (size_t)nA * XS * 4, hipMemcpyDeviceToDevice, s));
  } else if (!m.rec_emb_layers.empty()) {
    c.rec_node_enc = dalloc<float>(m, nullptr, {nR, XS}, true);
    DDMI_CHECK_HIP(hipMemcpyAsync(c.rec_node_enc, c.rec_node_base, (size_t)nR * XS * 4, hipMemcpyDeviceToDevice, s));
    std::vector<int> tgt_local(c.Err);
    for (int e = 0; e < c.Err; ++e) tgt_local[e] = rr_tgt[e] - c.nL;
    int* tl = m.cpool.upload(tgt_local);
    float* xa = dalloc<float>(m, nullptr, {nR, XS}, true);
    float* xin = c.rec_node_base;
    for (size_t i = 0; i < m.rec_emb_layers.size(); ++i) {
      const ConvW& L = m.rec_emb_layers[i];
      RunGroup g{0, nR, 0, nR, c.rr_goff, tl, c.rr_tslot, c.rr_arow, c.rec_edge_base, c.Err, nullptr, nullptr, nullptr,
                 c.rr_nvec, c.rr_ew, 1.f, c.msg[2]};
      g.vn = 1;
      float* xout = (xin == c.rec_node_base) ? xa : c.rec_node_base;
      run_conv(m, L, {g}, c.rg_rr, 1, xin, xout, 0, nR, s);
      xin = xout;
      c.rec_base_dim = L.D_out;
    }
    if (xin != c.rec_node_base)
      DDMI_CHECK_HIP(hipMemcpyAsync(c.rec_node_base, xin, (size_t)nR * XS * 4, hipMemcpyDeviceToDevice, s));
  }
  DDMI_CHECK_HIP(hipStreamSynchronize(s));
  m.has_complex = true;
}

static void score_readouts(Model& m, const float* XL, const float* lig_pos, const float* t_tr, const float* t_rot,
                           const float* t_tor, float* tr_out, float* rot_out, float* tor_out, hipStream_t s) {
  Cx& c = *m.cx;
  const ddmi_config& cfg = m.cfg;
  const int ns = m.ns, sd = m.sd, B = c.B, nL = c.nL;
  if (m.two_streams && m.side_stream && c.nT > 0 && tor_out) {
    DDMI_CHECK_HIP(hipEventRecord(m.ev_fork, s));
    DDMI_CHECK_HIP(hipStreamWaitEvent(m.side_stream, m.ev_fork, 0));
  }
  const ConvW& F = m.final_conv;
  launch_center_prep(lig_pos, c.lig_batch, c.lig_ptr, nL, cfg.sh_lmax, XL, cfg.fixed_center_conv ? c.c_xrow : c.lig_batch, ns, c.c_dist,
                     c.c_nvec, c.c_sh, F.sh_dim, c.c_attr, F.n_edge, s);
  {
    EdgeMlpArgs ea = mlp_args(m.center_edge, ns, nL, nullptr, c.c_dist, m.off_center, m.D, m.coeff_center, 0, c.center_gvec, c.lig_batch, c.c_attr);
    ea.ldo = F.n_edge;
    launch_edge_mlp(ea, s);
  }
  run_direct_conv(m, F, c.c_attr, nL, c.c_hid, c.c_W, c.c_xrow, XL, c.c_sh, nullptr, nullptr, 0, c.c_out, s);
  launch_segment_mean_bn(c.c_out, F.D_out, c.lig_ptr, nullptr, 0, B, F.D_out, F.has_bn ? F.bn_mean : nullptr,
                         F.has_bn ? F.bn_scale : nullptr, F.has_bn ? F.bn_bias : nullptr, c.gp, F.D_out, s);
  {
    ScoreHeadArgs a{};
    a.B = B; a.gp = c.gp; a.odd_parity = cfg.odd_parity; a.scale_by_sigma = cfg.scale_by_sigma; a.ns = ns; a.ldw0 = 1 + sd;
    a.tr_w0n = m.tr_final.W0; a.tr_sig = c.tr_sig; a.tr_w3 = m.tr_final.W3; a.tr_b3 = m.tr_final.b3;
    a.rot_w0n = m.rot_final.W0; a.rot_sig = c.rot_sig; a.rot_w3 = m.rot_final.W3; a.rot_b3 = m.rot_final.b3;
    a.t_tr = t_tr; a.t_rot = t_rot; a.tr_smin = cfg.tr_sigma_min; a.tr_smax = cfg.tr_sigma_max;
    a.rot_smin = cfg.rot_sigma_min; a.rot_smax = cfg.rot_sigma_max; a.so3_table = m.so3_table; a.so3_n = m.so3_n;
    a.tr_out = tr_out; a.rot_out = rot_out;
    launch_score_heads(a, s);
  }
  if (c.nT > 0 && tor_out) {
    const ConvW& T = m.tor_conv;
    const hipStream_t s_main = s;
    const bool fork = m.two_streams && m.side_stream;
    if (fork) s = m.side_stream;
    launch_tor_radius(lig_pos, c.lig_ptr, c.tor_u, c.tor_v, c.tor_batch, c.nT, cfg.lig_max_radius, c.tor_cap,
                      cfg.smooth_edges ? cfg.lig_max_radius : 0.f, c.t_cnt, c.t_atom, c.t_dist, c.t_nvec, c.t_ew, c.t_bond_nvec, s);
    {
      EdgeMlpArgs ea = mlp_args(m.final_edge, ns, c.Et, nullptr, c.t_dist, m.off_lig, m.D, m.coeff_lig, 0, m.final_edge.b0, nullptr, c.t_attr);
      ea.ldo = T.n_edge;
      launch_edge_mlp(ea, s);
    }
    launch_tor_prep(c.t_nvec, c.t_bond_nvec, c.nT, c.tor_cap, cfg.sh_lmax, m.tor_T, m.tor_ds, m.tor_dts, c.t_sh, XL, c.t_atom, c.tor_eu,
                    c.tor_ev, ns, c.t_attr, T.n_edge, s);
    run_direct_conv(m, T, c.t_attr, c.Et, c.t_hid, c.t_W, c.t_atom, XL, c.t_sh, c.t_ew, c.t_cnt, c.tor_cap, c.t_out, s);
    launch_segment_mean_bn(c.t_out, T.D_out, nullptr, c.t_cnt, c.tor_cap, c.nT, T.D_out, T.has_bn ? T.bn_mean : nullptr,
                           T.has_bn ? T.bn_scale : nullptr, T.has_bn ? T.bn_bias : nullptr, c.t_feat, T.D_out, s);
    TorHeadArgs a{};
    a.nT = c.nT; a.ns = ns; a.in_dim = T.D_out; a.feat = c.t_feat; a.W0 = m.tor_W0; a.W3 = m.tor_W3;
    a.tor_batch = c.tor_batch; a.t_tor = t_tor; a.smin = cfg.tor_sigma_min; a.smax = cfg.tor_sigma_max;
    a.scale_by_sigma = cfg.scale_by_sigma; a.torus_table = m.torus_table; a.torus_n = m.torus_n; a.out = tor_out;
    launch_tor_head(a, s);
    if (fork) {
      DDMI_CHECK_HIP(hipEventRecord(m.ev_join, m.side_stream));
      DDMI_CHECK_HIP(hipStreamWaitEvent(s_main, m.ev_join, 0));
    }
  }
}

static void forward_old(Model& m, const float* lig_pos, const float* t_tr, const float* t_rot, const float* t_tor, float* tr_out,
                        float* rot_out, float* tor_out, float* conf_out, hipStream_t s) {
  Cx& c = *m.cx;
  const ddmi_config& cfg = m.cfg;
  const int ns = m.ns, sd = m.sd, B = c.B, nL = c.nL, nR = c.nR, Lc = cfg.num_conv_layers;
  ++c.epoch;
  PhaseTimer t_fwd(m, "forward_total", s);
  std::unique_ptr<PhaseTimer> t_phase(new PhaseTimer(m, "embed_and_graphs", s));
  launch_time_embedding(t_tr, B, m.time_freq, sd / 2, cfg.embedding_scale, cfg.embedding_type, c.temb, s);
  gemm(c.temb, sd, m.old_lig_lin.W0, sd, m.old_lig_lin.b0, c.ligsig, ns, B, ns, sd, 0, s);
  if (m.lm > 0) gemm(c.temb, sd, m.old_lm_W + ns + m.lm - sd, ns + m.lm, nullptr, c.rec_sig, ns, B, ns, sd, 0, s);
  else gemm(c.temb, sd, m.old_rec_lin.W0, sd, m.old_rec_lin.b0, c.rec_sig, ns, B, ns, sd, 0, s);
  gemm(c.temb, sd, m.lig_edge.W0 + m.nf, m.lig_edge.in, m.lig_edge.b0, c.ll_gvec, ns, B, ns, sd, 0, s);
  gemm(c.temb, sd, m.cross_edge.W0, m.cross_edge.in, m.cross_edge.b0, c.cross_gvec, ns, B, ns, sd, 0, s);
  gemm(c.temb, sd, m.rec_edge.W0, m.rec_edge.in, m.rec_edge.b0, c.rr_sig_old, ns, B, ns, sd, 0, s);
  const bool conf = cfg.confidence_mode != 0;
  if (!conf) {
    gemm(c.temb, sd, m.center_edge.W0 + m.D, m.center_edge.in, m.center_edge.b0, c.center_gvec, ns, B, ns, sd, 0, s);
    gemm(c.temb, sd, m.tr_final.W0 + 1, 1 + sd, m.tr_final.b0, c.tr_sig, ns, B, ns, sd, 0, s);
    gemm(c.temb, sd, m.rot_final.W0 + 1, 1 + sd, m.rot_final.b0, c.rot_sig, ns, B, ns, sd, 0, s);
  }
// ... 191 lines not shown
  if (crop && !m.rec_emb_layers.empty()) {
    launch_add_rowvec(c.X[0] + (size_t)nL * XS, XS, c.rec_node_enc, XS, nullptr, 0, nullptr, nR, ns, 0, s);
    RunGroup g_rr0{nL, nR, nL, nR, c.goff2, c.tgt2, c.tslot2, c.arow2, c.rec_edge_base, c.Err, nullptr, nullptr,
                   nullptr, c.rr_nvec, c.rr_ew, 1.f, c.msg[2]};
    g_rr0.vn = 1;
    for (size_t i = 0; i < m.rec_emb_layers.size(); ++i)
      run_conv(m, m.rec_emb_layers[i], {g_rr0}, c.rg_rr_crop, 1, c.X[i], c.X[i + 1], nL, nR, s);
    launch_add_rowvec(c.X[xi] + (size_t)nL * XS, XS, c.X[xi] + (size_t)nL * XS, XS, c.rec_sig, ns, c.rec_batch, nR,
                      c.rec_base_dim, ns, s);
  } else if (!nodes_on_side) {
    launch_add_rowvec(c.X[xi] + (size_t)nL * XS, XS, c.rec_node_base, XS, c.rec_sig, ns, c.rec_batch, nR, c.rec_base_dim, ns, s);
  }
  if (early_cross) DDMI_CHECK_HIP(hipStreamWaitEvent(s, m.ev_cross, 0));
  else cross_graph(s, keep);
  RunGroup g_lr{nL, nR, 0, nL, c.offs_r, c.g1_tgt, c.g1_tslot, c.g1_tslot, c.cross_ea, c.Elr_cap, c.offs_l + nL, nullptr,
                      nullptr, c.pnvec, c.pew, 1.f, c.msg[1]};
  RunGroup g_rr{nL, nR, nL, nR, crop ? c.goff2 : c.rr_goff, crop ? c.tgt2 : c.rr_tgt, crop ? c.tslot2 : c.rr_tslot,
                      crop ? c.arow2 : c.rr_arow, c.rec_edge_base, c.Err, nullptr, c.rec_sig, c.rr_batch, c.rr_nvec, c.rr_ew,
                      1.f, c.msg[2]};
  RunGroup g_rl{0, nL, nL, nR, c.offs_l, c.g3_tgt, c.g3_tslot, nullptr, c.cross_ea, c.Elr_cap, c.offs_l + nL, nullptr,
                nullptr, c.pnvec, c.pew, -1.f, c.msg[3]};
  g_lr.vn = 0; g_rr.vn = 1; g_rl.vn = 3; g_rl.load = true;
  g_rr.static_topo = !crop;
  const int Lc = (int)m.conv_layers.size();
  if (cfg.all_atoms) {
    const int nA = c.nA, aB = nL + nR;
    launch_add_rowvec(c.X[xi] + (size_t)aB * XS, XS, c.atom_node_base, XS, c.rec_sig, ns, c.atom_batch, nA, c.rec_base_dim, ns, s);
    launch_cross_count(lig_pos, c.atom_pos, c.lig_batch, c.atom_batch, c.lig_ptr, c.atom_ptr, nL, nA, c.maxNa, nullptr,
                       cfg.lig_max_radius, nullptr, c.la_pairrank, c.la_cnt_l, c.la_cnt_a, s);
    launch_exclusive_scan2(c.la_cnt_l, c.la_offs_l, nL, c.la_cnt_a, c.la_offs_a, nA, s);
    launch_cross_fill(lig_pos, c.atom_pos, c.atom_batch, c.lig_ptr, c.atom_ptr, nL, nA, c.maxNa, c.la_pairrank, c.la_offs_l,
                      c.la_offs_a, nullptr, cfg.lig_max_radius, cfg.smooth_edges, c.la1_tgt, c.la1_tslot, c.la3_tgt, c.la3_tslot,
                      c.la_pbatch, c.la_dist, c.la_nvec, c.la_ew, s, aB);
    gemm(c.temb, sd, m.la_edge.W0, m.la_edge.in, m.la_edge.b0, c.la_gvec, ns, B, ns, sd, 0, s);
    launch_edge_mlp(mlp_args(m.la_edge, ns, c.Ela_cap, c.la_offs_l + nL, c.la_dist, m.off_lig, m.D, m.coeff_lig, sd, c.la_gvec,
                             c.la_pbatch, c.la_ea), s);
    RunGroup a_ll = g_ll, a_lr = g_lr, a_rr = g_rr, a_rl = g_rl;
    a_rl.sgn = 1.f;
    a_ll.msg = c.msg_aa[0]; a_lr.msg = c.msg_aa[1]; a_rr.msg = c.msg_aa[3]; a_rl.msg = c.msg_aa[4];
    RunGroup a_la{aB, nA, 0, nL, c.la_offs_a, c.la1_tgt, c.la1_tslot, c.la1_tslot, c.la_ea, c.Ela_cap, c.la_offs_l + nL, nullptr,
                  nullptr, c.la_nvec, c.la_ew, 1.f, c.msg_aa[2]};
    RunGroup a_ra{aB, nA, nL, nR, c.se_ra.goff, c.se_ra.tgt, c.se_ra.tslot, c.se_ra.arow, c.ar_edge_base, c.Ear, nullptr, c.rec_sig,
                  c.ar_batch, c.ar_nvec, nullptr, 1.f, c.msg_aa[5]};
    RunGroup a_aa{aB, nA, aB, nA, c.se_aa.goff, c.se_aa.tgt, c.se_aa.tslot, c.se_aa.arow, c.atom_edge_base, c.Eaa, nullptr, c.rec_sig,
                  c.aa_batch, c.aa_nvec, c.aa_ew, 1.f, c.msg_aa[6]};
    RunGroup a_al{0, nL, aB, nA, c.la_offs_l, c.la3_tgt, c.la3_tslot, nullptr, c.la_ea, c.Ela_cap, c.la_offs_l + nL, nullptr,
                  nullptr, c.la_nvec, c.la_ew, 1.f, c.msg_aa[7]};
    RunGroup a_ar{nL, nR, aB, nA, c.se_ar.goff, c.se_ar.tgt, c.se_ar.tslot, c.se_ar.arow, c.ar_edge_base, c.Ear, nullptr, c.rec_sig,
                  c.ar_batch, c.ar_nvec, nullptr, 1.f, c.msg_aa[8]};
    a_la.vn = 4; a_ra.vn = 5; a_aa.vn = 6; a_al.vn = 7; a_al.load = true; a_ar.vn = 8;
    a_ra.static_topo = a_aa.static_topo = a_ar.static_topo = true;
    t_phase.reset();
    for (int l = 0; l < Lc; ++l, ++xi) {
      if (l < Lc - 1)
        run_conv(m, m.conv_layers[l], {a_ll, a_lr, a_la, a_rr, a_rl, a_ra, a_aa, a_al, a_ar}, c.rg_aa_all, 9, c.X[xi], c.X[xi + 1], 0,
                 c.N, s);
      else run_conv(m, m.conv_layers[l], {a_ll, a_lr, a_la}, c.rg_aa_lig, 3, c.X[xi], c.X[xi + 1], 0, nL, s);
    }
  } else {
    t_phase.reset();
    bool overlapped = m.layer_overlap && m.two_streams && m.side_stream && nR > 0 && Lc >= 2;
    if (overlapped) {
      long biggest = 1;
      for (const RunGroup* q : {&g_ll, &g_lr, &g_rr, &g_rl}) biggest = std::max(biggest, tiles_of(*q));
      overlapped = biggest >= 256 || m.layer_overlap == 2;
    }
    bool nu = m.node_update && !overlapped && Lc >= 2 && m.fused_mm && ns % 16 == 0 && ns <= 64 && c.Pg[0] && (int)c.rb_l.size() == Lc;
    for (auto& L : m.conv_layers) {
      nu = nu && L.TL == 2 && L.H == m.conv_layers[0].H && L.n_edge == m.conv_layers[0].n_edge;
      for (int g = 0; g < 4; ++g) nu = nu && L.W1p[std::min(g, L.G - 1)];
    }
    if (nu) {
      PhaseTimer t(m, "conv_fc1_gemms", s);
      GemmBatch gb;
      for (int l = 0; l < Lc - 1; ++l) {
        const ConvW& L = m.conv_layers[l];
        if (gb.n == GEMM_BATCH_MAX) { launch_gemm_batch(gb, s); gb.n = 0; }
        GemmArgs& x = gb.g[gb.n++];
        x = GemmArgs{};
        x.A = c.rec_sig; x.lda = ns; x.W = L.W1p[std::min(2, L.G - 1)]; x.ldw = L.n_edge; x.C = c.rb_l[l]; x.ldc = L.H; x.M = B; x.N = L.H; x.K = ns;
      }
      if (gb.n) launch_gemm_batch(gb, s);
    }
    if (overlapped) run_conv_layers_overlapped(m, g_ll, g_lr, g_rr, g_rl, crop ? c.rg_all_crop : c.rg_all, xi, s);
    else
    for (int l = 0; l < Lc; ++l, ++xi) {
      RunGroup rr = g_rr;
      if (nu && l < Lc - 1) rr.rb_ready = c.rb_l[l];
      const std::vector<RunGroup> full = {g_ll, g_lr, rr, g_rl}, ligs = {g_ll, g_lr};
      std::vector<RunGroup> next;
      if (nu && l + 1 < Lc) {
        if (l + 1 < Lc - 1) next = {g_ll, g_lr, g_rr, g_rl}; else next = ligs;
      }
      const int pq = !nu ? 0 : l == 0 ? 1 : 2;
      const ConvW* Ln = next.empty() ? nullptr : &m.conv_layers[l + 1];
      if (l < Lc - 1)
        run_conv(m, m.conv_layers[l], full, crop ? c.rg_all_crop : c.rg_all, 4, c.X[xi], c.X[xi + 1], 0, c.N, s, pq, Ln, Ln ? &next : nullptr);
      else run_conv(m, m.conv_layers[l], ligs, c.rg_lig, 2, c.X[xi], c.X[xi + 1], 0, cfg.sidechain_pred ? c.N : nL, s, pq);
    }
  }
  const float* XL = c.X[xi];
  c.x_last = conf ? nullptr : XL;
  PhaseTimer t_read(m, "readouts", s);
  if (conf) {
    const int total = cfg.num_conv_layers + cfg.num_prot_emb_layers;
    const ConvW& Ll = m.conv_layers.back();
    ConfHeadArgs a{};
    a.B = B; a.X = XL; a.ldx = XS; a.col0 = 0; a.lig_ptr = c.lig_ptr; a.ns = ns;
    a.n_tail = total >= 3 ? (cfg.reduce_pseudoscalars ? cfg.nv : ns) : 0;
    a.tail_off = Ll.D_out - a.n_tail;
    if (cfg.atom_confidence) {
      const int n_in = ns + a.n_tail, na = cfg.atom_num_confidence_outputs, wo = na + ns;
      launch_gather_cols(c.ac_in, n_in, 0, XL, XS, nullptr, nL, ns, nullptr, s);
      if (a.n_tail > 0) launch_gather_cols(c.ac_in, n_in, ns, XL + a.tail_off, XS, nullptr, nL, a.n_tail, nullptr, s);
      gemm(c.ac_in, n_in, m.aconf_W[0], n_in, m.aconf_b[0], c.ac_h0, ns, nL, ns, n_in, 1, s);
      gemm(c.ac_h0, ns, m.aconf_W[1], ns, m.aconf_b[1], c.ac_h1, ns, nL, ns, ns, 1, s);
      gemm(c.ac_h1, ns, m.aconf_W[2], ns, m.aconf_b[2], c.ac_out, wo, nL, wo, ns, 0, s);
      launch_gather_cols(atom_conf_out, na, 0, c.ac_out, wo, nullptr, nL, na, nullptr, s);
      a.X = c.ac_out; a.ldx = wo; a.col0 = na; a.n_tail = 0; a.tail_off = 0;
    }
    a.W0 = m.conf_W[0]; a.b0 = m.conf_b[0]; a.sc0 = m.conf_bn_scale[0]; a.sh0 = m.conf_bn_shift[0];
    a.W1 = m.conf_W[1]; a.b1 = m.conf_b[1]; a.sc1 = m.conf_bn_scale[1]; a.sh1 = m.conf_bn_shift[1];
    a.W2 = m.conf_W[2]; a.b2 = m.conf_b[2]; a.n_out = cfg.num_confidence_outputs + (cfg.affinity_prediction ? 1 : 0); a.out = conf_out;
    launch_conf_head(a, s);
    return;
  }
  score_readouts(m, XL, lig_pos, t_tr, t_rot, t_tor, tr_out, rot_out, tor_out, s);
}

void sidechain_pred(Model& m, float* out, hipStream_t s) {
  DDMI_REQUIRE(m.has_complex && m.cx->x_last && m.side_Mt, DDMI_ERR_STATE,
               "ddmi_sidechain_pred reads the node table of the ddmi_forward directly before it (none since the last ddmi_confidence / ddmi_sample / ddmi_set_complex)");
  Cx& c = *m.cx;
  gemm(c.x_last + (size_t)c.nL * XS, XS, m.side_Mt, m.side_K, nullptr, out, 10, c.nR, 10, m.side_K, 0, s);
}

void modify_conformer(Model& m, float* lig_pos, const float* tr, const float* rot, const float* tor, hipStream_t s) {
  DDMI_REQUIRE(m.has_complex, DDMI_ERR_STATE, "ddmi_set_complex must precede ddmi_modify_conformer");
  Cx& c = *m.cx;
  DDMI_REQUIRE(c.uniform && c.Nl_one > 0, DDMI_ERR_STATE,
               "modify_conformer needs a batch of copies of one complex (utils/diffusion_utils.py:60-64)");
  const bool torsion = tor != nullptr && c.R_one > 0;
  DDMI_REQUIRE(!torsion || c.mask_rotate, DDMI_ERR_STATE, "mask_rotate was not provided to ddmi_set_complex");
  launch_modify_conformer(lig_pos, c.B, c.Nl_one, torsion ? c.R_one : 0, c.rot_u, c.rot_v, c.mask_rotate, tr, rot,
                          torsion ? tor : nullptr, s);
}

static const long long* upload_sample_ids(Model& m, const int64_t* ids, hipStream_t s) {
  Cx& c = *m.cx;
  if (!ids) return nullptr;
  if (!c.s_ids) {
    c.s_ids = m.cpool.alloc<long long>(c.B);
    DDMI_CHECK_HIP(hipHostMalloc(reinterpret_cast<void**>(&c.s_ids_host), (size_t)c.B * 8));
    DDMI_CHECK_HIP(hipEventCreate(&c.s_ids_ev));
  } else {
    DDMI_CHECK_HIP(hipEventSynchronize(c.s_ids_ev));
  }
  for (int b = 0; b < c.B; ++b) c.s_ids_host[b] = ids[b];
  DDMI_CHECK_HIP(hipMemcpyAsync(c.s_ids, c.s_ids_host, (size_t)c.B * 8, hipMemcpyHostToDevice, s));
  DDMI_CHECK_HIP(hipEventRecord(c.s_ids_ev, s));
  return c.s_ids;
}

static void perturb_step(Model& m, float* tr, float* rot, float* tor, const ddmi_sample_cfg& sc, int k,
                         const long long* ids_dev, hipStream_t s) {
  Cx& c = *m.cx;
  const ddmi_config& cfg = m.cfg;
  const int steps = sc.inference_steps, B = c.B;
  const bool torsion = tor != nullptr && !cfg.no_torsion && c.nT > 0;
  const bool last = k == steps - 1;
  const double t_tr = sc.tr_schedule[k], t_rot = sc.rot_schedule[k], t_tor = sc.tor_schedule[k];
  const double dt_tr = last ? t_tr : t_tr - sc.tr_schedule[k + 1];
  const double dt_rot = last ? t_rot : t_rot - sc.rot_schedule[k + 1];
  const double dt_tor = last ? t_tor : t_tor - sc.tor_schedule[k + 1];
  const double s_tr = std::pow((double)cfg.tr_sigma_min, 1 - t_tr) * std::pow((double)cfg.tr_sigma_max, t_tr);
  const double s_rot = std::pow((double)cfg.rot_sigma_min, 1 - t_rot) * std::pow((double)cfg.rot_sigma_max, t_rot);
  const double s_tor = std::pow((double)cfg.tor_sigma_min, 1 - t_tor) * std::pow((double)cfg.tor_sigma_max, t_tor);
  const bool zero_noise = sc.no_random || (sc.no_final_step_noise && last) || sc.ode;
  auto coeffs = [&](double sigma, double smin, double smax, double dt, int i, float& cs, float& cz) {
    const double g = sigma * std::sqrt(2.0 * std::log(smax / smin));
    double a = sc.ode ? 0.5 * g * g * dt : g * g * dt;
    double z = g * std::sqrt(dt);
    if (sc.temp_sampling[i] != 1.0) {
      const double T = sc.temp_sampling[i], psi = sc.temp_psi[i], sdat = sc.temp_sigma_data[i];
      const double sigma_data = std::exp(sdat * std::log(smax) + (1 - sdat) * std::log(smin));
      const double lambda = (sigma_data + sigma) / (sigma_data + sigma / T);
      a = g * g * dt * (lambda + T * psi / 2);
      z = g * std::sqrt(dt * (1 + psi));
    }
    cs = (float)a;
    cz = zero_noise ? 0.f : (float)z;
  };
  PerturbArgs p{};
  p.B = B; p.R = torsion ? c.nT / B : 0; p.tr = tr; p.rot = rot; p.tor = tor;
  coeffs(s_tr, cfg.tr_sigma_min, cfg.tr_sigma_max, dt_tr, 0, p.c_tr_s, p.c_tr_z);
  coeffs(s_rot, cfg.rot_sigma_min, cfg.rot_sigma_max, dt_rot, 1, p.c_rot_s, p.c_rot_z);
  coeffs(s_tor, cfg.tor_sigma_min, cfg.tor_sigma_max, dt_tor, 2, p.c_tor_s, p.c_tor_z);
  if (!zero_noise) {
    p.z_tr = sc.z_tr ? sc.z_tr + (size_t)k * B * 3 : nullptr;
    p.z_rot = sc.z_rot ? sc.z_rot + (size_t)k * B * 3 : nullptr;
    p.z_tor = sc.z_tor ? sc.z_tor + (size_t)k * c.nT : nullptr;
    p.use_rng = 1;
  }
  p.seed = sc.seed; p.sample_ids = ids_dev; p.step = k;
  launch_perturb(p, s);
}

static void check_sample_cfg(Model& m, const ddmi_sample_cfg& sc) {
  DDMI_REQUIRE(sc.inference_steps > 0 && sc.tr_schedule && sc.rot_schedule && sc.tor_schedule, DDMI_ERR_ARG, "bad schedule");
  DDMI_REQUIRE(m.cx->uniform, DDMI_ERR_STATE, "the step loop needs a batch of copies of one complex");
}

void perturb(Model& m, float* tr, float* rot, float* tor, const ddmi_sample_cfg& sc, int k, hipStream_t s) {
  DDMI_REQUIRE(m.has_complex, DDMI_ERR_STATE, "ddmi_set_complex must precede ddmi_perturb");
  check_sample_cfg(m, sc);
  DDMI_REQUIRE(k >= 0 && k < sc.inference_steps, DDMI_ERR_ARG, "step index out of range");
  perturb_step(m, tr, rot, tor, sc, k, upload_sample_ids(m, sc.sample_ids, s), s);
}

void sample(Model& m, float* lig_pos, const ddmi_sample_cfg& sc, hipStream_t s) {
  DDMI_REQUIRE(m.has_complex, DDMI_ERR_STATE, "ddmi_set_complex must precede ddmi_sample");
  check_sample_cfg(m, sc);
  Cx& c = *m.cx;
  const ddmi_config& cfg = m.cfg;
  const int steps = sc.inference_steps, B = c.B;
  const bool torsion = !cfg.no_torsion && c.nT > 0;
  struct CropGuard {
    Model& m; double saved;
    ~CropGuard() { m.crop_cutoff = saved; }
  } crop_guard{m, m.crop_cutoff};
  if (!c.s_t) c.s_t = m.cpool.alloc<float>((size_t)3 * B * STEP_TIMES_MAX);
  const long long* ids_dev = upload_sample_ids(m, sc.sample_ids, s);
  const bool times_once = steps <= STEP_TIMES_MAX;
  if (times_once) {
    StepTimes st{};
    st.steps = steps;
    for (int k = 0; k < steps; ++k) { st.t[3 * k] = (float)sc.tr_schedule[k]; st.t[3 * k + 1] = (float)sc.rot_schedule[k]; st.t[3 * k + 2] = (float)sc.tor_schedule[k]; }
    launch_fill_times_all(c.s_t, B, st, s);
  }
  for (int k = 0; k < steps; ++k) {
    const double t_tr = sc.tr_schedule[k], t_rot = sc.rot_schedule[k], t_tor = sc.tor_schedule[k];
    const double s_tr = std::pow((double)cfg.tr_sigma_min, 1 - t_tr) * std::pow((double)cfg.tr_sigma_max, t_tr);
    float* tk = times_once ? c.s_t + (size_t)k * 3 * B : c.s_t;
    if (!times_once) launch_fill_times(tk, B, (float)t_tr, (float)t_rot, (float)t_tor, s);
    m.crop_cutoff = sc.use_crop ? s_tr * 3.0 + sc.crop_beyond : 0.0;
    forward(m, lig_pos, tk, tk + B, tk + 2 * B, c.s_tr, c.s_rot, torsion ? c.s_tor : nullptr, s);
    perturb_step(m, c.s_tr, c.s_rot, torsion ? c.s_tor : nullptr, sc, k, ids_dev, s);
#ifdef DDMI_PROFILING
    static const bool freeze = getenv("DDMI_FREEZE_POSE") != nullptr;
#else
    constexpr bool freeze = false;
#endif
    if (!freeze) modify_conformer(m, lig_pos, c.s_tr, c.s_rot, torsion ? c.s_tor : nullptr, s);
  }
  c.x_last = nullptr;
}

}
```

diffdock_amd/csrc/k_conv.hip:

```cpp
#include "k_conv_tile.h"

namespace ddmi {

__global__ void k_vn_count(const int* __restrict__ goff, int gcount, int* __restrict__ cnt) {
  const int d = blockIdx.x * blockDim.x + threadIdx.x;
  if (d >= gcount) return;
  cnt[d] = (goff[d + 1] - goff[d] + 31) >> 5;
}
__global__ void k_vn_fill(const int* __restrict__ goff, const int* __restrict__ voff, int gcount, int* __restrict__ vn_node,
                          int* __restrict__ vn_e0) {
  const int d = blockIdx.x * blockDim.x + threadIdx.x;
  if (d >= gcount) return;
  const int v0 = voff[d], n = voff[d + 1] - v0, e0 = goff[d], e1 = goff[d + 1];
  for (int b = 0; b < n; ++b) { vn_node[v0 + b] = d; vn_e0[v0 + b] = min(e0 + 32 * b, e1); }
}
__global__ void k_vn_fill_pp(const int* __restrict__ goff, const int* __restrict__ voff, int gcount, const int* __restrict__ node_batch,
                             const int* __restrict__ graph_ptr, int n_graphs, int* __restrict__ vn_node, int* __restrict__ vn_e0,
                             int* __restrict__ nvn_pad) {
  const int d = blockIdx.x * blockDim.x + threadIdx.x;
  if (d >= gcount) return;
  const int b = node_batch[d];
  int pad = 0;
  for (int q = 0; q < b; ++q) { const int n = voff[graph_ptr[q + 1]] - voff[graph_ptr[q]]; pad += ((n + 15) & ~15) - n; }
  const int v0 = voff[d] + pad, n = voff[d + 1] - voff[d], e0 = goff[d], e1 = goff[d + 1];
// ... 204 lines not shown
    h[4 + tid] = (pre && k != 0x7fffffff) ? rw[((size_t)(v0 + (k >> 5)) * 32 + (k & 31)) * 8 + 5] : -1;
  }
  if (tid == 0) { h[0] = pre ? 1 : 0; h[1] = t0; h[2] = pre ? nt : 0; h[3] = 0; }
}
void launch_vn_tiles(const int* nvn, int vcap, const float* vrows, const int* vn_ne, int* tile_hdr, unsigned char* live, hipStream_t s) {
  if (vcap <= 0) return;
  hipLaunchKernelGGL(k_vn_tiles, dim3(cdiv(vcap, 16)), dim3(256), 0, s, nvn, vrows, vn_ne, tile_hdr, live);
  DDMI_CHECK_HIP(hipGetLastError());
}

static_assert(FC_VN == 16, "k_vn_rows pads the per-edge rows to whole 16-node tiles");

#define FC_EXTERN(MAXD, SHD, MODE, NBK, BF) extern template void launch_conv_fused_k<MAXD, SHD, MODE, NBK, BF>(const FusedConvArgs&, hipStream_t);
FC_EXTERN(3, 4, 1, 4, false) FC_EXTERN(3, 4, 0, 4, false) FC_EXTERN(3, 4, 3, 4, false) FC_EXTERN(3, 4, 4, 4, false)
FC_EXTERN(3, 4, 0, 5, false) FC_EXTERN(3, 4, 3, 5, false) FC_EXTERN(3, 4, 4, 5, false)
FC_EXTERN(3, 4, 0, 4, true) FC_EXTERN(3, 4, 3, 4, true) FC_EXTERN(3, 4, 4, 4, true)
FC_EXTERN(3, 4, 0, 5, true) FC_EXTERN(3, 4, 3, 5, true) FC_EXTERN(3, 4, 4, 5, true)
FC_EXTERN(3, 9, 1, 4, false) FC_EXTERN(3, 9, 0, 4, false) FC_EXTERN(3, 9, 3, 4, false)
FC_EXTERN(5, 9, 1, 4, false) FC_EXTERN(5, 9, 0, 4, false) FC_EXTERN(5, 9, 3, 4, false)
#undef FC_EXTERN
#ifdef DDMI_PROFILING
void fc_prof_report_f32(); void fc_prof_report_bf(); void fc_prof_report_l2(); void fc_prof_report_grp();
void fc_prof_report() { fc_prof_report_f32(); fc_prof_report_bf(); fc_prof_report_l2(); fc_prof_report_grp(); }
#endif

void launch_conv_fused(const FusedConvArgs& a_in, hipStream_t s) {
  if (a_in.vcap <= 0 || a_in.ysplit <= 0) return;
  FusedConvArgs a = a_in;
  a.dbg = ablate_mask();
#ifdef FCV_QUICK
  launch_conv_fused_k<3, 4, 3, 4, true>(a, s);
  return;
#endif
  if (a.tile_hdr && (a.generic || a.shared || a.maxd > 3 || a.sh_lmax > 1))
    throw Error(DDMI_ERR_STATE, "k_conv_fused: pre-reduced group routed to a kernel variant without the pre-reducing epilogue");
  if (a.generic && a.max_nb > 4) throw Error(DDMI_ERR_ARG, "k_conv_fused: packed granule in a generic layer (weights.cpp builds those layers unpacked)");
  if (a.maxd <= 3 && a.sh_lmax <= 1) {
    if (a.bf && a.generic) throw Error(DDMI_ERR_ARG, "k_conv_fused: bf16 edge product requested for a generic layer (complex.cpp falls back to f32 there)");
    if (a.generic) launch_conv_fused_k<3, 4, 1, 4>(a, s);
    else if (a.bf && a.max_nb > 4) {
      if (a.dense && a.shared) launch_conv_fused_k<3, 4, 4, 5, true>(a, s);
      else if (a.dense) launch_conv_fused_k<3, 4, 3, 5, true>(a, s);
      else launch_conv_fused_k<3, 4, 0, 5, true>(a, s);
    } else if (a.bf) {
      if (a.dense && a.shared) launch_conv_fused_k<3, 4, 4, 4, true>(a, s);
      else if (a.dense) launch_conv_fused_k<3, 4, 3, 4, true>(a, s);
      else launch_conv_fused_k<3, 4, 0, 4, true>(a, s);
    } else if (a.max_nb > 4) {
      if (a.dense && a.shared) launch_conv_fused_k<3, 4, 4, 5>(a, s);
      else if (a.dense) launch_conv_fused_k<3, 4, 3, 5>(a, s);
      else launch_conv_fused_k<3, 4, 0, 5>(a, s);
    } else {
      if (a.dense && a.shared) launch_conv_fused_k<3, 4, 4, 4>(a, s);
      else if (a.dense) launch_conv_fused_k<3, 4, 3, 4>(a, s);
      else launch_conv_fused_k<3, 4, 0, 4>(a, s);
    }
  } else if (a.bf) {
    throw Error(DDMI_ERR_ARG, "k_conv_fused: bf16 edge product requested with sh_lmax > 1 (complex.cpp falls back to f32 there)");
  } else if (a.maxd <= 3) {
    if (a.generic) launch_conv_fused_k<3, 9, 1, 4>(a, s);
    else if (a.dense) launch_conv_fused_k<3, 9, 3, 4>(a, s);
    else launch_conv_fused_k<3, 9, 0, 4>(a, s);
  } else {
    if (a.generic) launch_conv_fused_k<5, 9, 1, 4>(a, s);
    else if (a.dense) launch_conv_fused_k<5, 9, 3, 4>(a, s);
    else launch_conv_fused_k<5, 9, 0, 4>(a, s);
  }
}

__global__ __launch_bounds__(256) void k_reduce_bn(const ReduceGroup* __restrict__ groups, int n_groups, int nbase,
                                                   int D_in, int D_out, const float* __restrict__ bn_mean,
                                                   const float* __restrict__ bn_scale, const float* __restrict__ bn_bias,
                                                   int residual, const float* __restrict__ X_in,
                                                   float* __restrict__ X_out, int out_stride) {
  __shared__ float red[4][XS + 4];
  const int s = nbase + blockIdx.x;
  const int tid = threadIdx.x, lane = tid & 63;
  const int wave = DDMI_UNIFORM(tid >> 6);
  const bool live = 4 * lane < D_out;
  float4 acc = make_float4(0.f, 0.f, 0.f, 0.f);
  int cnt = 0;
  for (int g = 0; g < n_groups; ++g) {
    const ReduceGroup G = groups[g];
    const int sl = s - G.tbase;
    if (sl < 0 || sl >= G.tcount) continue;
    const int b = G.toff[sl], e = G.toff[sl + 1];
    cnt += e - b;
    if (G.live) {
      const float* __restrict__ mp = G.msg + 4 * lane;
      int ord = 0;
      for (int base = b; base < e; base += 64) {
        const int rr = base + lane;
        unsigned long long mask = __ballot(rr < e && G.live[rr] != 0);
        while (mask) {
          int rows[4];
#pragma unroll
          for (int i = 0; i < 4; ++i) {
            rows[i] = -1;
            while (mask && rows[i] < 0) {
              const int bit = __builtin_ctzll(mask);
              mask &= mask - 1;
              if ((ord++ & 3) == wave) rows[i] = base + bit;
            }
          }
          float4 v[4];
#pragma unroll
          for (int i = 0; i < 4; ++i) v[i] = (live && rows[i] >= 0) ? nt_load4(mp + (size_t)rows[i] * XS) : make_float4(0.f, 0.f, 0.f, 0.f);
#pragma unroll
          for (int i = 0; i < 4; ++i)
            if (rows[i] >= 0) { acc.x += v[i].x; acc.y += v[i].y; acc.z += v[i].z; acc.w += v[i].w; }
        }
      }
    } else if (live) {
      const float* __restrict__ mp = G.msg + 4 * lane;
      int r = b + wave;
      for (; r + 12 < e; r += 16) {
        const float4 v0 = nt_load4(mp + (size_t)r * XS), v1 = nt_load4(mp + (size_t)(r + 4) * XS);
        const float4 v2 = nt_load4(mp + (size_t)(r + 8) * XS), v3 = nt_load4(mp + (size_t)(r + 12) * XS);
        acc.x += v0.x; acc.y += v0.y; acc.z += v0.z; acc.w += v0.w;
        acc.x += v1.x; acc.y += v1.y; acc.z += v1.z; acc.w += v1.w;
        acc.x += v2.x; acc.y += v2.y; acc.z += v2.z; acc.w += v2.w;
        acc.x += v3.x; acc.y += v3.y; acc.z += v3.z; acc.w += v3.w;
      }
      for (; r < e; r += 4) {
        const float4 v0 = nt_load4(mp + (size_t)r * XS);
        acc.x += v0.x; acc.y += v0.y; acc.z += v0.z; acc.w += v0.w;
      }
    }
  }
  if (4 * lane < XS) *reinterpret_cast<float4*>(&red[wave][4 * lane]) = acc;
  __syncthreads();
  const int c = tid;
  if (c >= out_stride) return;
  float v = 0.f;
  if (c < D_out) {
    const float sum = (red[0][c] + red[1][c]) + (red[2][c] + red[3][c]);
    v = cnt > 0 ? sum / (float)cnt : 0.f;
    if (bn_scale) v = (v - bn_mean[c]) * bn_scale[c] + bn_bias[c];
    if (residual && c < D_in) v += X_in[(size_t)s * XS + c];
  }
  X_out[(size_t)s * out_stride + c] = v;
}

void launch_reduce_bn(const ReduceGroup* groups_dev, int n_groups, int nbase, int ncount, int D_in, int D_out,
                      const float* bn_mean, const float* bn_scale, const float* bn_bias, int residual,
                      const float* X_in, float* X_out, int out_stride, hipStream_t s) {
  if (ncount <= 0) return;
  hipLaunchKernelGGL(k_reduce_bn, dim3(ncount), dim3(256), 0, s, groups_dev, n_groups, nbase, D_in, D_out, bn_mean,
                     bn_scale, bn_bias, residual, X_in, X_out, out_stride);
  DDMI_CHECK_HIP(hipGetLastError());
}

}
```

diffdock_amd/csrc/k_graph.hip:

```cpp
#include "kernels.h"

namespace ddmi {

__device__ __forceinline__ float dist2_rn(float ax, float ay, float az, float bx, float by, float bz) {
#ifdef DDMI_HIPEMU
  volatile float dx = ax - bx, dy = ay - by, dz = az - bz;
  volatile float xx = dx * dx, yy = dy * dy, zz = dz * dz;
  volatile float s = xx + yy;
  return s + zz;
#else
  const float dx = __fsub_rn(ax, bx), dy = __fsub_rn(ay, by), dz = __fsub_rn(az, bz);
  return __fadd_rn(__fadd_rn(__fmul_rn(dx, dx), __fmul_rn(dy, dy)), __fmul_rn(dz, dz));
#endif
}

__global__ __launch_bounds__(1024) void k_exclusive_scan(const int* __restrict__ in, int* __restrict__ out, int n) {
  __shared__ int part[1024];
  const int t = threadIdx.x;
  const int per = (n + 1023) / 1024;
  const int lo = min(t * per, n), hi = min(lo + per, n);
  int s = 0;
  for (int i = lo; i < hi; ++i) s += in[i];
  part[t] = s;
  __syncthreads();
// ... 177 lines not shown
    const int j = ((int)blockIdx.x - lig_blocks) * 256 + threadIdx.x;
    if (j >= nR) return;
    const int b = rbatch[j], lo = lptr[b], hi = lptr[b + 1];
    const float cut = cutoff ? cutoff[b] : const_cutoff;
    int c = 0;
    if (!keep || keep[j])
      for (int i = lo; i < hi; ++i) c += cross_in_range(lpos + 3 * i, rpos + 3 * j, cut, cutoff != nullptr);
    cnt_r[j] = c;
  }
}
void launch_cross_count(const float* lpos, const float* rpos, const int* lbatch, const int* rbatch, const int* lptr,
                        const int* rptr, int nL, int nR, int maxNr, const float* cutoff, float const_cutoff,
                        const int* keep, int* pairrank, int* cnt_l, int* cnt_r, hipStream_t s) {
  if (nL + nR <= 0) return;
  hipLaunchKernelGGL(k_cross_count, dim3(cdiv(nL, 4) + cdiv(nR, 256)), dim3(256), 0, s, lpos, rpos, lbatch, rbatch, lptr, rptr, nL,
                     nR, maxNr, cutoff, const_cutoff, keep, pairrank, cnt_l, cnt_r);
  DDMI_CHECK_HIP(hipGetLastError());
}

__global__ void k_cross_fill(const float* __restrict__ lpos, const float* __restrict__ rpos,
                             const int* __restrict__ rbatch, const int* __restrict__ lptr, const int* __restrict__ rptr,
                             int nL, int nR, int maxNr, const int* __restrict__ pairrank, const int* __restrict__ offs_l,
                             const int* __restrict__ offs_r, const float* __restrict__ cutoff, float const_cutoff,
                             int smooth, int* __restrict__ g1_tgt, int* __restrict__ g1_tslot, int* __restrict__ g3_tgt,
                             int* __restrict__ g3_tslot, int* __restrict__ pbatch, float* __restrict__ pdist,
                             float* __restrict__ pnvec, float* __restrict__ pew, int rbase) {
  const int j = blockIdx.x * blockDim.x + threadIdx.x;
  if (j >= nR) return;
  const int b = rbatch[j], lo = lptr[b], hi = lptr[b + 1], jl = j - rptr[b];
  const float cut = cutoff ? cutoff[b] : const_cutoff;
  int rr = 0;
  for (int i = lo; i < hi; ++i) {
    const int rl = pairrank[(size_t)i * maxNr + jl];
    if (rl < 0) continue;
    const int e_l = offs_l[i] + rl, e_r = offs_r[j] + rr++;
    g1_tgt[e_r] = i;
    g1_tslot[e_r] = e_l;
    g3_tgt[e_l] = rbase + j;
    g3_tslot[e_l] = e_r;
    pbatch[e_l] = b;
    write_geom(rpos[3 * j] - lpos[3 * i], rpos[3 * j + 1] - lpos[3 * i + 1], rpos[3 * j + 2] - lpos[3 * i + 2],
               smooth ? cut : 0.f, e_l, pdist, pnvec, pew);
  }
}
void launch_cross_fill(const float* lpos, const float* rpos, const int* rbatch, const int* lptr, const int* rptr, int nL,
                       int nR, int maxNr, const int* pairrank, const int* offs_l, const int* offs_r, const float* cutoff,
                       float const_cutoff, int smooth, int* g1_tgt, int* g1_tslot, int* g3_tgt, int* g3_tslot,
                       int* pbatch, float* pdist, float* pnvec, float* pew, hipStream_t s, int rbase) {
  if (nR <= 0) return;
  hipLaunchKernelGGL(k_cross_fill, dim3(cdiv(nR, 64)), dim3(64), 0, s, lpos, rpos, rbatch, lptr, rptr, nL, nR, maxNr,
                     pairrank, offs_l, offs_r, cutoff, const_cutoff, smooth, g1_tgt, g1_tslot, g3_tgt, g3_tslot, pbatch,
                     pdist, pnvec, pew, rbase < 0 ? nL : rbase);
  DDMI_CHECK_HIP(hipGetLastError());
}

__global__ void k_cross_cutoff(const float* __restrict__ t_tr, int B, float smin, float smax, float* __restrict__ out, int raw) {
  const int b = blockIdx.x * blockDim.x + threadIdx.x;
  if (b >= B) return;
  const float sigma = raw ? t_tr[b] : powf(smin, 1.f - t_tr[b]) * powf(smax, t_tr[b]);
  out[b] = sigma * 3.f + 20.f;
}
void launch_cross_cutoff(const float* t_tr, int B, float smin, float smax, float* out, hipStream_t s, int raw) {
  hipLaunchKernelGGL(k_cross_cutoff, dim3(cdiv(B, 64)), dim3(64), 0, s, t_tr, B, smin, smax, out, raw);
  DDMI_CHECK_HIP(hipGetLastError());
}

__global__ void k_crop_mask(const float* __restrict__ lpos, const float* __restrict__ rpos, const int* __restrict__ rbatch,
                            const int* __restrict__ lptr, int nR, float cut2, int* __restrict__ keep) {
  const int j = blockIdx.x * blockDim.x + threadIdx.x;
  if (j >= nR) return;
  const int b = rbatch[j];
  int k = 0;
  for (int i = lptr[b]; i < lptr[b + 1] && !k; ++i)
    k = dist2_rn(lpos[3 * i], lpos[3 * i + 1], lpos[3 * i + 2], rpos[3 * j], rpos[3 * j + 1], rpos[3 * j + 2]) < cut2;
  keep[j] = k;
}
void launch_crop_mask(const float* lpos, const float* rpos, const int* rbatch, const int* lptr, int nR, float cut2, int* keep,
                      hipStream_t s) {
  if (nR <= 0) return;
  hipLaunchKernelGGL(k_crop_mask, dim3(cdiv(nR, 64)), dim3(64), 0, s, lpos, rpos, rbatch, lptr, nR, cut2, keep);
  DDMI_CHECK_HIP(hipGetLastError());
}

__global__ void k_rr_filter_count(const int* __restrict__ keep, const int* __restrict__ goff, const int* __restrict__ tgt,
                                  const int* __restrict__ toff, const int* __restrict__ tlist,
                                  const int* __restrict__ gnode, int nL, int nR, int* __restrict__ cnt_g,
                                  int* __restrict__ cnt_t) {
  const int n = blockIdx.x * blockDim.x + threadIdx.x;
  if (n >= nR) return;
  int cg = 0, ct = 0;
  if (keep[n]) {
    for (int e = goff[n]; e < goff[n + 1]; ++e) cg += keep[tgt[e] - nL];
    for (int ts = toff[n]; ts < toff[n + 1]; ++ts) ct += keep[gnode[tlist[ts]]];
  }
  cnt_g[n] = cg;
  cnt_t[n] = ct;
}
__global__ void k_rr_filter_tslot(const int* __restrict__ keep, const int* __restrict__ toff, const int* __restrict__ tlist,
                                  const int* __restrict__ gnode, const int* __restrict__ toff2, int nR,
                                  int* __restrict__ tslot_tmp) {
  const int n = blockIdx.x * blockDim.x + threadIdx.x;
  if (n >= nR || !keep[n]) return;
  int r = toff2[n];
  for (int ts = toff[n]; ts < toff[n + 1]; ++ts) {
    const int e = tlist[ts];
    if (keep[gnode[e]]) tslot_tmp[e] = r++;
  }
}
__global__ void k_rr_filter_fill(const int* __restrict__ keep, const int* __restrict__ goff, const int* __restrict__ tgt,
                                 const int* __restrict__ arow, const int* __restrict__ tslot_tmp,
                                 const int* __restrict__ goff2, int nL, int nR, int* __restrict__ tgt2,
                                 int* __restrict__ tslot2, int* __restrict__ arow2) {
  const int n = blockIdx.x * blockDim.x + threadIdx.x;
  if (n >= nR || !keep[n]) return;
  int q = goff2[n];
  for (int e = goff[n]; e < goff[n + 1]; ++e)
    if (keep[tgt[e] - nL]) { tgt2[q] = tgt[e]; tslot2[q] = tslot_tmp[e]; arow2[q] = arow[e]; ++q; }
}
void launch_rr_filter(const int* keep, const int* goff, const int* tgt, const int* arow, const int* toff, const int* tlist,
                      const int* gnode, int nL, int nR, int* cnt_g, int* cnt_t, int* goff2, int* toff2, int* tslot_tmp,
                      int* tgt2, int* tslot2, int* arow2, hipStream_t s) {
  if (nR <= 0) return;
  const dim3 grid(cdiv(nR, 64)), block(64);
  hipLaunchKernelGGL(k_rr_filter_count, grid, block, 0, s, keep, goff, tgt, toff, tlist, gnode, nL, nR, cnt_g, cnt_t);
  launch_exclusive_scan(cnt_g, goff2, nR, s);
  launch_exclusive_scan(cnt_t, toff2, nR, s);
  hipLaunchKernelGGL(k_rr_filter_tslot, grid, block, 0, s, keep, toff, tlist, gnode, toff2, nR, tslot_tmp);
  hipLaunchKernelGGL(k_rr_filter_fill, grid, block, 0, s, keep, goff, tgt, arow, tslot_tmp, goff2, nL, nR, tgt2, tslot2, arow2);
  DDMI_CHECK_HIP(hipGetLastError());
}

__global__ void k_tor_radius(const float* __restrict__ pos, const int* __restrict__ ptr, const int* __restrict__ tor_u,
                             const int* __restrict__ tor_v, const int* __restrict__ tor_batch, int nT, float r2, int cap,
                             float smooth_max, int* __restrict__ cnt, int* __restrict__ atom, float* __restrict__ dist,
                             float* __restrict__ nvec, float* __restrict__ ew, float* __restrict__ bond_nvec) {
  const int t = blockIdx.x * blockDim.x + threadIdx.x;
  if (t >= nT) return;
  const int u = tor_u[t], v = tor_v[t], b = tor_batch[t];
  const float mx = (pos[3 * u] + pos[3 * v]) / 2, my = (pos[3 * u + 1] + pos[3 * v + 1]) / 2,
              mz = (pos[3 * u + 2] + pos[3 * v + 2]) / 2;
  {
    const float bx = pos[3 * v] - pos[3 * u], by = pos[3 * v + 1] - pos[3 * u + 1], bz = pos[3 * v + 2] - pos[3 * u + 2];
    const float inv = 1.f / fmaxf(sqrtf(bx * bx + by * by + bz * bz), 1e-12f);
    bond_nvec[3 * t] = bx * inv; bond_nvec[3 * t + 1] = by * inv; bond_nvec[3 * t + 2] = bz * inv;
  }
  int c = 0;
  for (int a = ptr[b]; a < ptr[b + 1] && c < cap; ++a) {
    if (dist2_rn(pos[3 * a], pos[3 * a + 1], pos[3 * a + 2], mx, my, mz) < r2) {
      const int e = t * cap + c++;
      atom[e] = a;
      write_geom(pos[3 * a] - mx, pos[3 * a + 1] - my, pos[3 * a + 2] - mz, smooth_max, e, dist, nvec, ew);
    }
  }
  cnt[t] = c;
  for (int q = c; q < cap; ++q) {
    const int e = t * cap + q;
    atom[e] = u;
    dist[e] = 0.f;
    nvec[3 * e] = nvec[3 * e + 1] = nvec[3 * e + 2] = 0.f;
    if (ew) ew[e] = 0.f;
  }
}
void launch_tor_radius(const float* pos, const int* ptr, const int* tor_u, const int* tor_v, const int* tor_batch, int nT,
                       float r, int cap, float smooth_max, int* cnt, int* atom, float* dist, float* nvec, float* ew,
                       float* bond_nvec, hipStream_t s) {
  if (nT <= 0) return;
// ... 7 lines not shown
```

diffdock_amd/csrc/kernels.h:

```cpp
#pragma once
#include "ddmi_common.h"

namespace ddmi {

struct GemmArgs {
  const float* A = nullptr; int lda = 0;
  const float* W = nullptr; int ldw = 0;
  const float* bias = nullptr;
  const float* rowbias = nullptr; const int* ridx = nullptr; int ldrb = 0;
  float* C = nullptr; int ldc = 0;
  int M = 0, N = 0, K = 0;
  const int* m_dev = nullptr;
  int act = 0;
};
void launch_gemm(const GemmArgs& a, hipStream_t s);
constexpr int GEMM_BATCH_MAX = 16;
struct GemmBatch { GemmArgs g[GEMM_BATCH_MAX]; int n = 0; };
void launch_gemm_batch(const GemmBatch& b, hipStream_t s);

struct ObInfo { int base, itemw, mul, o_off, dout; };
struct DevPath {
  int n_off, mul_out, din, ds, dout, s_off, c_off, o_off;
  int mul_in, i_off, w_off;
  int g_off;
// ... 28 lines not shown
  int vcap; float* rows; int* vn_ne;
  int* tile_hdr = nullptr; unsigned char* live = nullptr;
};
struct VnPoseTiles { const int* node_batch; const int* graph_ptr; int n_graphs; int* nvn_pad; };
void launch_vn_build(const int* goff, int gcount, int* cnt_tmp, int* voff, int* vn_node, int* vn_e0, const VnRowsArgs& rows,
                     hipStream_t s, const VnPoseTiles* pp = nullptr);
constexpr int VN_GROUPS_MAX = 9;
struct VnListArgs { const int* goff; int gcount; int* voff; int* vn_node; int* vn_e0;
                    const int* node_batch; const int* graph_ptr; int n_graphs; int* nvn_pad; };
struct VnListsArgs { int n = 0; VnListArgs g[VN_GROUPS_MAX]; };
struct VnRowsGroupedArgs { int n = 0; int first[VN_GROUPS_MAX + 1] = {}; VnRowsArgs g[VN_GROUPS_MAX]; };
static_assert(sizeof(VnRowsGroupedArgs) <= 2048 && sizeof(VnListsArgs) <= 2048, "kernel arguments");
void launch_vn_build_all(const VnListsArgs& lists, const VnRowsArgs* rows , int sh_lmax, hipStream_t s);
constexpr int FC_TILE_HDR = 36, FC_TILE_NT = 32;
void launch_vn_tiles(const int* nvn, int vcap, const float* vrows, const int* vn_ne, int* tile_hdr, unsigned char* live, hipStream_t s);
void launch_edge_hidden(const int* nvn, int vcap, const int* vn_node, const int* vn_e0, const int* goff, const int* arow,
                        const int* tgt, int tbase, const float* HE, const float* P, const float* Q, int H, int NG8,
                        float* Hb, hipStream_t s, int bf = 0);
void launch_edge_rows(const int* nvn, int vcap, const int* vn_node, const int* vn_e0, const int* goff, const int* arow,
                      const int* tgt, int tbase, const float* HE, const float* P, const float* Q, int H, float* rows, hipStream_t s);
struct EdgeHiddenArgs {
  const int* nvn; int vcap; const int* vn_node; const int* vn_e0; const int* goff;
  const int* arow; const int* tgt; int tbase;
  const float* ea; int ns;
  const float* W1; int ldw;
  const float* P;
  const float* Q;
  const float* rowbias; const int* ridx;
  int H, NG8;
  int zero_fill;
  const float* vrows; const int* vn_ne;
  float* Hb;
  int bf;
  int grid;
};
void launch_edge_hidden_mm(const EdgeHiddenArgs& a, hipStream_t s);
constexpr int EH_GROUPS_MAX = 4;
struct EdgeHiddenGroupedArgs {
  int n = 0;
  int first[EH_GROUPS_MAX + 1] = {};
  EdgeHiddenArgs g[EH_GROUPS_MAX];
};
void launch_edge_hidden_mm_grouped(const EdgeHiddenGroupedArgs& G, hipStream_t s);

struct FusedConvArgs {
  const int* nvn; int vcap;
  const int* vn_node;
  const float* vrows; const int* vn_ne;
  const float* X; int gbase;
  const float* wpack; int KS, HK;
  const float* Hb; int NG8;
  int sh_lmax;
  const FGran* gran; int ysplit; int gsplit[9];
  const float* cgt;
  int max_nb;
  int maxd;
  int generic;
  int dense;
  int shared;
  int n_units; short ustart[48];
  short ufirst[8], ucount[8];
  float* msg;
  const int* tile_hdr = nullptr;
  int bf = 0;
  int dbg = 0;
  int prof_slot = 0;
};
#if defined(DDMI_PROFILING)
void fc_prof_report();
#endif
void launch_conv_fused(const FusedConvArgs& a, hipStream_t s);

constexpr int FC_GROUPS_MAX = 4;
struct FusedGroupedArgs {
  int n = 0;
  int first[FC_GROUPS_MAX + 1] = {};
  int ntile[FC_GROUPS_MAX] = {};
  int mode[FC_GROUPS_MAX] = {};
  FusedConvArgs g[FC_GROUPS_MAX];
};
static_assert(sizeof(FusedGroupedArgs) <= 3072, "kernel arguments of k_conv_grouped (4 KB limit)");
void launch_conv_grouped(const FusedGroupedArgs& G, hipStream_t s);

struct ReduceGroup { const int* toff; const float* msg; int tbase, tcount; const unsigned char* live = nullptr; };
void launch_reduce_bn(const ReduceGroup* groups_dev, int n_groups, int nbase, int ncount, int D_in, int D_out,
                      const float* bn_mean, const float* bn_scale, const float* bn_bias, int residual,
                      const float* X_in, float* X_out, int out_stride, hipStream_t s);

constexpr int NU_TERMS_MAX = 8;
struct NodeTerm { const float* W; const float* bias; float* out; int base, count; };
struct NodeUpdateArgs {
  const ReduceGroup* groups; int n_groups, nbase, ncount, D_in, D_out;
  const float *bn_mean, *bn_scale, *bn_bias; int residual;
  const float* X_in; float* X_out;
  int n_terms; NodeTerm term[NU_TERMS_MAX];
  int ns, H, ldw;
  int wpn;
};
void launch_node_update(const NodeUpdateArgs& a, hipStream_t s);

void launch_exclusive_scan(const int* in, int* out, int n, hipStream_t s);
void launch_exclusive_scan2(const int* in0, int* out0, int n0, const int* in1, int* out1, int n1, hipStream_t s);
void launch_lig_radius(const float* pos, const int* batch, const int* ptr, int nL, int maxNl, float r, int cap,
                       int* adjrank, int* cnt_g, hipStream_t s);
void launch_ll_count(const int* adjrank, const int* batch, const int* ptr, int nL, int maxNl, const int* bg,
                     const int* bt, int* cnt_g_inout, int* cnt_t, hipStream_t s);
void launch_ll_fill(const float* pos, const int* batch, const int* ptr, int nL, int maxNl, const int* adjrank,
                    const int* goff, const int* toff, const int* bg, const int* bt, int n_bonds, const int* bond_src,
                    const int* bond_dst, const int* bond_grank, const int* bond_trank, float smooth_max,
                    int* tgt, int* tslot, int* featidx, int* ebatch, float* dist, float* nvec, float* ew, hipStream_t s);
void launch_cross_count(const float* lpos, const float* rpos, const int* lbatch, const int* rbatch, const int* lptr,
                        const int* rptr, int nL, int nR, int maxNr, const float* cutoff, float const_cutoff,
                        const int* keep, int* pairrank, int* cnt_l, int* cnt_r, hipStream_t s);
void launch_crop_mask(const float* lpos, const float* rpos, const int* rbatch, const int* lptr, int nR, float cut2, int* keep,
                      hipStream_t s);
void launch_rr_filter(const int* keep, const int* goff, const int* tgt, const int* arow, const int* toff, const int* tlist,
                      const int* gnode, int nL, int nR, int* cnt_g, int* cnt_t, int* goff2, int* toff2, int* tslot_tmp,
                      int* tgt2, int* tslot2, int* arow2, hipStream_t s);
void launch_cross_fill(const float* lpos, const float* rpos, const int* rbatch, const int* lptr, const int* rptr, int nL,
                       int nR, int maxNr, const int* pairrank, const int* offs_l, const int* offs_r, const float* cutoff,
                       float const_cutoff, int smooth, int* g1_tgt, int* g1_tslot, int* g3_tgt, int* g3_tslot,
                       int* pbatch, float* pdist, float* pnvec, float* pew, hipStream_t s,
                       int rbase = -1 );
void launch_cross_cutoff(const float* t_tr, int B, float smin, float smax, float* out, hipStream_t s, int raw = 0);
void launch_tor_radius(const float* pos, const int* ptr, const int* tor_u, const int* tor_v, const int* tor_batch, int nT,
                       float r, int cap, float smooth_max, int* cnt, int* atom, float* dist, float* nvec, float* ew,
                       float* bond_nvec, hipStream_t s);

void launch_time_embedding(const float* t, int B, const float* freq, int half, float scale, int fourier, float* out, hipStream_t s);
constexpr int TIME_TERMS_MAX = 8;
struct TimeTermsArgs {
  const float* t; int B; const float* freq; int half; float scale; int fourier; float* temb;
  int ns, n;
  struct { const float* W; int ldw; const float* bias; float* C; int act; } term[TIME_TERMS_MAX];
  int hid_term; const float* W3; const float* b3; float* out3;
};
void launch_time_terms(const TimeTermsArgs& a, hipStream_t s);
void launch_lig_node_embed(const int* x, int nL, const float* emb, const int* emb_off, int n_feat, int ns, float* out,
                           hipStream_t s);
void launch_add_rowvec(float* X, int ldx, const float* base, int ldb, const float* vec, int ldv, const int* idx, int rows,
                       int cols, int zero_to, hipStream_t s);
struct EdgeMlpArgs {
  int E = 0; const int* e_dev = nullptr;
  const float* dist = nullptr;
  const float* offsets = nullptr; int D = 0; float coeff = 0;
  const float* feat = nullptr; const int* featidx = nullptr; int nfeat = 0;
  const float* W0f = nullptr; int ldw0f = 0;
  const float* W0g = nullptr; int ldw0g = 0;
  const float* gvec = nullptr; const int* gidx = nullptr;
  const float* W1 = nullptr; const float* b1 = nullptr;
  int ns = 0;
  float* out = nullptr; int ldo = 0;
};
void launch_edge_mlp(const EdgeMlpArgs& a, hipStream_t s);
void launch_rec_edge_geom(const float* pos, const int* src, const int* dst, int E, float smooth_max, float* dist,
                          float* nvec, float* ew, hipStream_t s, const float* pos_dst = nullptr);
void launch_add3(float* out, const float* x, int d_in, const float* u1, const float* u2, int rows, int d_out, hipStream_t s);
void launch_concat_rec_input(const float* rec_x, int ldx, const float* emb, int ns, int lm, int nR, float* out,
                             hipStream_t s);

void launch_center_prep(const float* pos, const int* batch, const int* ptr, int nL, int lmax, const float* X, const int* xrow, int ns,
                        float* dist, float* nvec, float* sh, int lds_, float* attr, int lda, hipStream_t s);
void launch_tor_prep(const float* edge_nvec, const float* bond_nvec, int nT, int cap, int lmax, const float* T, int ds, int dts, float* out,
                     const float* X, const int* atom, const int* eu, const int* ev, int ns, float* attr, int lda, hipStream_t s);
void launch_center_edges(const float* pos, const int* batch, const int* ptr, int B, int nL, float* dist, float* nvec,
                         hipStream_t s);
void launch_sh_rows(const float* nvec, float sgn, int E, int lmax, float* sh, int lds, hipStream_t s);
void launch_tor_sh(const float* edge_nvec, const float* bond_nvec, int nT, int cap, int lmax, const float* T, int ds,
                   int dts, float* out, hipStream_t s);
void launch_gather_cols(float* dst, int ldd, int col0, const float* src, int lds_, const int* rowidx, int rows, int cols,
                        const int* rowidx2, hipStream_t s);
struct TpApplyArgs {
  int E; const int* valid_cnt; int cap;
  const float* Wt; int ldw;
  const float* X; const int* xrow;
  const float* sh; int lds_;
  const float* ew;
  const DevPath* paths; const float* ctab; const CgItem* items; int n_items;
  int n_paths, z_floats;
  int form = -1;
  float* out; int ldo;
};
void launch_tp_apply(const TpApplyArgs& a, hipStream_t s);
void launch_segment_mean_bn(const float* rows, int ldr, const int* seg_off, const int* seg_cnt, int cap, int n_seg,
                            int D, const float* bn_mean, const float* bn_scale, const float* bn_bias, float* out,
                            int ldo, hipStream_t s);
struct ScoreHeadArgs {
  int B; const float* gp;
  int odd_parity, scale_by_sigma, ns, ldw0;
  const float *tr_w0n, *tr_sig, *tr_w3, *tr_b3;
  const float *rot_w0n, *rot_sig, *rot_w3, *rot_b3;
  const float *t_tr, *t_rot;
  float tr_smin, tr_smax, rot_smin, rot_smax;
  const float* so3_table; int so3_n;
  float *tr_out, *rot_out;
};
void launch_score_heads(const ScoreHeadArgs& a, hipStream_t s);
struct ConfHeadArgs {
// ... 36 lines not shown
```

diffdock_amd/csrc/model.h:

```cpp
#pragma once
#include <map>
#include <memory>
#include <string>
#include <vector>

#include "kernels.h"
#include "o3_host.h"

namespace ddmi {

struct HostTensor {
  std::vector<float> data;
  std::vector<int64_t> shape;
  int64_t numel() const { int64_t n = 1; for (auto d : shape) n *= d; return n; }
};

class DevicePool {
 public:
  ~DevicePool();
  void* alloc_bytes(size_t n);
  template <class T> T* alloc(size_t n) { return reinterpret_cast<T*>(alloc_bytes(n * sizeof(T))); }
  template <class T> T* upload(const std::vector<T>& v) {
    T* p = alloc<T>(v.size() ? v.size() : 1);
    if (!v.empty()) DDMI_CHECK_HIP(hipMemcpy(p, v.data(), v.size() * sizeof(T), hipMemcpyHostToDevice));
// ... 11 lines not shown
  int G = 1;
  bool faster = false, residual = true, has_bn = true, yform = true;
  Irreps in_irr, sh_irr, out_irr;
  TPTable table;
  int n_edge = 0, H = 0, HK = 0, D_in = 0, D_out = 0, NT = 0, sh_dim = 0, Wn = 0;
  bool depthwise = false; int Wn_dw = 0, n_lin2 = 0;
  std::vector<float*> W1, b1, W2, b2, wpack;
  int TL = 2;
  std::vector<std::vector<float*>> Wmid, bmid;
  std::vector<float*> W1p, b1p;
  int KS = 0;
  FGran* fgran = nullptr; int n_fgran = 0, HKq = 0; bool fgran_generic = false;
  float* cgt = nullptr; int max_nb = 4;
  std::vector<int> fgran_unit;
  int maxd = 1;
  DevPath* paths = nullptr; float* ctab = nullptr; CgItem* items = nullptr; int n_items = 0;
  float *bn_mean = nullptr, *bn_scale = nullptr, *bn_bias = nullptr;
};

struct Mlp2W { float *W0 = nullptr, *b0 = nullptr, *W3 = nullptr, *b3 = nullptr; int in = 0, hid = 0, out = 0; };

struct DebugEntry { const void* ptr; std::vector<int64_t> shape; bool is_int; };

struct Model {
  ddmi_config cfg{};
  int device = 0;
  std::vector<std::pair<std::string, std::vector<int64_t>>> spec;
  std::map<std::string, HostTensor> host_w;
  bool committed = false;
  DevicePool wpool, tpool;
  int ns = 0, sd = 0, D = 0, Dc = 0, nf = 0, lm = 0, H = 0;
  float* lig_emb = nullptr; int* lig_emb_off = nullptr;
  Mlp2W lig_enc;
  Mlp2W lig_edge, rec_edge, rec_sigma, cross_edge, center_edge, final_edge, tr_final, rot_final;
  Mlp2W atom_edge, ar_edge, la_edge;
  float* atom_emb = nullptr; int* atom_emb_off = nullptr;
  float *conf_W[3] = {}, *conf_b[3] = {}, *conf_bn_scale[2] = {}, *conf_bn_shift[2] = {};
  float *aconf_W[3] = {}, *aconf_b[3] = {};
  float* rec_emb = nullptr; float *rec_enc_W = nullptr, *rec_enc_b = nullptr;
  float *off_lig = nullptr, *off_rec = nullptr, *off_cross = nullptr, *off_center = nullptr;
  float coeff_lig = 0, coeff_rec = 0, coeff_cross = 0, coeff_center = 0;
  std::vector<ConvW> rec_emb_layers, lig_emb_layers, conv_layers;
  ConvW final_conv, tor_conv;
  std::vector<ConvW> old_lig, old_rec, old_l2r, old_r2l;
  Mlp2W old_lig_lin, old_rec_lin;
  float *old_lm_W = nullptr, *old_lm_b = nullptr;
  float *tor_W0 = nullptr, *tor_W3 = nullptr;
  float* side_Mt = nullptr; int side_K = 0;
  float* tor_T = nullptr; int tor_ds = 0, tor_dts = 0;
  float* time_freq = nullptr;
  std::vector<float> time_freq_host;
  float *so3_table = nullptr, *torus_table = nullptr; int so3_n = 0, torus_n = 0;
  bool has_complex = false;
  hipStream_t side_stream = nullptr;
  hipEvent_t ev_fork = nullptr, ev_join = nullptr, ev_cross = nullptr, ev_terms = nullptr;
  bool two_streams = true;
  int layer_overlap = 0;
  std::vector<hipEvent_t> ev_pipe;
  int fused_shared = 1;
  bool fused_tri = true;
  bool fused_pack = true;
  int tp_form = -1;
  bool fc1_batch = true;
  bool fused_mm = true;
  int fused_dense = 1;
  bool fused_prered = true;
  int fused_ysplit = 0;
  int fused_ysplit_small = 0;
  bool tight_caps = false;
  bool time_terms_fused = false;
  int group_order = 0;
  bool ys_rounds_small = false;
  bool ys_rounds = true;
  int n_cus = 256;
  int fused_ysplit_last = 0;
  int eh_grid = 2048;
  int grouped = 0;
  int grouped_split = 0;
  int grouped_target = 1536;
  int node_update_wpn = 0;
  bool node_update = false;
  bool vn_merge = true;
  bool tile_per_pose = false;
  double crop_cutoff = 0.0;
  DevicePool cpool;
  struct Cx;
  std::shared_ptr<Cx> cx;
  std::map<std::string, DebugEntry> debug;
  bool timing = false;
  int timing_level = 0;
  struct TimedPhase { std::string name; double ms = 0; int64_t launches = 0; };
  std::vector<TimedPhase> phases;
  struct EventPair { int phase; hipEvent_t a, b; };
  std::vector<EventPair> pending;
  std::vector<hipEvent_t> free_events;
};

struct PhaseTimer {
  Model& m; hipStream_t s; int idx = -1; hipEvent_t a{}, b{};
  PhaseTimer(Model& model, const char* name, hipStream_t stream);
  ~PhaseTimer();
};
void resolve_timings(Model& m);

void build_weight_spec(Model& m);
void commit_weights(Model& m);
void set_complex(Model& m, const ddmi_complex& c, hipStream_t s);
void forward(Model& m, const float* lig_pos, const float* t_tr, const float* t_rot, const float* t_tor, float* tr_out,
             float* rot_out, float* tor_out, hipStream_t s, float* conf_out = nullptr, float* atom_conf_out = nullptr);
void modify_conformer(Model& m, float* lig_pos, const float* tr, const float* rot, const float* tor, hipStream_t s);
void sidechain_pred(Model& m, float* out, hipStream_t s);
void sample(Model& m, float* lig_pos, const ddmi_sample_cfg& sc, hipStream_t s);
void perturb(Model& m, float* tr, float* rot, float* tor, const ddmi_sample_cfg& sc, int k, hipStream_t s);

}
```

diffdock_amd/lib.py:

```python
from __future__ import annotations

import ctypes as C
import os
import subprocess

import numpy as np

CSRC = os.path.join(os.path.dirname(os.path.abspath(__file__)), "csrc")
DEFAULT_LIB = os.path.join(CSRC, "libddmi.so")


class DdmiError(RuntimeError):
    pass


EDGE_PRODUCTS = {"f32": 0, "bf16x4": 1}


class ExecOptions(C.Structure):
    _fields_ = [(n, C.c_int32) for n in ("streams", "dense_rows", "shared_tiles", "packed_granules", "merged_granule", "pre_reduce",
                                         "hidden_mm", "fc1_batch", "tile_split", "tile_split_small", "hidden_grid", "tp_apply",
                                         "debug", "tile_per_pose", "layer_overlap", "grouped", "grouped_split", "vn_build", "node_update", "tile_split_last", "tile_split_rule", "group_order", "list_caps", "time_terms")]


def harness_enabled() -> bool:
    return os.environ.get("DDMI_HARNESS") == "1"


def _env_int(name):
    v = os.environ.get(name)
    if v is None or v == "":
        return None
    try:
        return int(v)
    except ValueError:
        raise DdmiError(f"{name}: integer expected, got '{v}'") from None


def exec_options_from_env(base=()) -> ExecOptions:
    x = ExecOptions()
    for k, v in dict(base or ()).items():
        setattr(x, k, int(v))
    if not harness_enabled():
        return x
    e = _env_int
    if e("DDMI_STREAMS") is not None: x.streams = 1 if e("DDMI_STREAMS") == 1 else 0
    for var, field in (("DDMI_FUSED_DENSE", "dense_rows"), ("DDMI_FUSED_SHARED", "shared_tiles")):
        if e(var) is not None:
            if e(var) not in (0, 1, 2):
                raise DdmiError(f"{var}: 0 (never), 1 (default rule) or 2 (always)")
            setattr(x, field, {1: 0, 0: 1, 2: 2}[e(var)])
    for var, field in (("DDMI_FUSED_PACK", "packed_granules"), ("DDMI_FUSED_TRI", "merged_granule"), ("DDMI_FUSED_PRERED", "pre_reduce"),
                       ("DDMI_FUSED_MM", "hidden_mm"), ("DDMI_FC1_BATCH", "fc1_batch")):
        if e(var) is not None: setattr(x, field, 0 if e(var) != 0 else 1)
    if e("DDMI_FUSED_YS") is not None: x.tile_split = max(0, e("DDMI_FUSED_YS"))
    if e("DDMI_TIME_TERMS") is not None: x.time_terms = 1 if e("DDMI_TIME_TERMS") else 0
    if e("DDMI_LIST_CAPS") is not None: x.list_caps = 1 if e("DDMI_LIST_CAPS") else 0
    if e("DDMI_GROUP_ORDER") is not None: x.group_order = max(0, min(3, e("DDMI_GROUP_ORDER")))
    if e("DDMI_YS_RULE") is not None: x.tile_split_rule = max(0, min(2, e("DDMI_YS_RULE")))
    if e("DDMI_FUSED_YS_LAST") is not None: x.tile_split_last = max(0, min(8, e("DDMI_FUSED_YS_LAST")))
    if e("DDMI_FUSED_YS_SMALL") is not None: x.tile_split_small = max(0, e("DDMI_FUSED_YS_SMALL"))
    if e("DDMI_EH_GRID") is not None: x.hidden_grid = max(0, e("DDMI_EH_GRID"))
    tp = os.environ.get("DDMI_TP_APPLY")
    if tp is not None:
        if tp not in ("auto", "wave", "edge", "thread"):
            raise DdmiError(f"DDMI_TP_APPLY: unknown form '{tp}' (wave | edge | thread | auto)")
        x.tp_apply = {"auto": 0, "wave": 1, "edge": 2, "thread": 3}[tp]
    if os.environ.get("DDMI_DEBUG_GRAN"): x.debug = 1
    if e("DDMI_TILE_PER_POSE") is not None: x.tile_per_pose = 1 if e("DDMI_TILE_PER_POSE") else 0
    if e("DDMI_LAYER_OVERLAP") is not None:
        if e("DDMI_LAYER_OVERLAP") not in (0, 1, 2):
            raise DdmiError("DDMI_LAYER_OVERLAP: 0 (joined layers), 1 (chip-filling batches) or 2 (always)")
        x.layer_overlap = e("DDMI_LAYER_OVERLAP")
    if e("DDMI_NODE_UPDATE") is not None: x.node_update = max(0, min(3, e("DDMI_NODE_UPDATE")))
    if e("DDMI_VN_BUILD") is not None: x.vn_build = 1 if e("DDMI_VN_BUILD") else 0
    if e("DDMI_GROUPED") is not None:
        if e("DDMI_GROUPED") not in (0, 1, 2):
            raise DdmiError("DDMI_GROUPED: 0 / 1 (per-group launches) or 2 (grouped)")
        x.grouped = e("DDMI_GROUPED")
    if e("DDMI_GROUPED_YS") is not None: x.grouped_split = max(0, min(8, e("DDMI_GROUPED_YS")))
    return x


class Config(C.Structure):
    _fields_ = [("struct_size", C.c_uint32)] + \
               [(n, C.c_int32) for n in ("ns", "nv", "num_conv_layers", "num_prot_emb_layers", "sh_lmax",
                                         "sigma_embed_dim", "distance_embed_dim", "cross_distance_embed_dim",
                                         "in_lig_edge_features", "lm_embedding_dim")] + \
               [(n, C.c_float) for n in ("lig_max_radius", "rec_max_radius", "cross_max_distance", "center_max_distance")] + \
               [(n, C.c_int32) for n in ("dynamic_max_cross", "use_second_order_repr", "reduce_pseudoscalars",
                                         "differentiate_convolutions", "embed_also_ligand", "batch_norm", "smooth_edges",
                                         "odd_parity", "no_torsion", "scale_by_sigma", "fixed_center_conv")] + \
               [(n, C.c_float) for n in ("embedding_scale", "tr_sigma_min", "tr_sigma_max", "rot_sigma_min",
                                         "rot_sigma_max", "tor_sigma_min", "tor_sigma_max")] + \
               [("all_atoms", C.c_int32), ("confidence_mode", C.c_int32), ("num_confidence_outputs", C.c_int32),
                ("old_model", C.c_int32), ("atom_confidence", C.c_int32), ("atom_num_confidence_outputs", C.c_int32),
                ("affinity_prediction", C.c_int32), ("embedding_type", C.c_int32), ("tp_weights_layers", C.c_int32),
                ("sidechain_pred", C.c_int32), ("depthwise_convolution", C.c_int32), ("edge_product", C.c_int32), ("exec", ExecOptions)]


class Complex(C.Structure):
    _fields_ = [(n, C.c_int32) for n in ("num_graphs", "n_lig", "n_rec", "n_bond_edges", "n_rec_edges", "n_tor")] + \
               [(n, C.c_void_p) for n in ("lig_ptr", "rec_ptr", "lig_x", "bond_index", "bond_attr", "edge_mask", "rec_x",
                                          "rec_pos", "rec_edge_index", "mask_rotate")] + \
               [(n, C.c_int32) for n in ("n_atom", "n_atom_edges", "n_atom_rec_edges")] + \
               [(n, C.c_void_p) for n in ("atom_ptr", "atom_x", "atom_pos", "atom_edge_index", "atom_rec_edge_index")]


class SampleCfg(C.Structure):
    _fields_ = [("inference_steps", C.c_int32), ("tr_schedule", C.c_void_p), ("rot_schedule", C.c_void_p),
                ("tor_schedule", C.c_void_p), ("ode", C.c_int32), ("no_random", C.c_int32),
                ("no_final_step_noise", C.c_int32), ("temp_sampling", C.c_double * 3), ("temp_psi", C.c_double * 3),
                ("temp_sigma_data", C.c_double * 3), ("seed", C.c_uint64), ("sample_ids", C.c_void_p),
                ("z_tr", C.c_void_p), ("z_rot", C.c_void_p), ("z_tor", C.c_void_p),
                ("use_crop", C.c_int32), ("crop_beyond", C.c_double)]


def make_config(cfg) -> Config:
    c = Config()
    for name, _ in Config._fields_:
        if name == "struct_size":
            c.struct_size = C.sizeof(Config)
        elif name == "lm_embedding_dim":
            c.lm_embedding_dim = cfg.lm_embedding_dim
        elif name == "old_model":
            c.old_model = int(cfg.old)
        elif name == "embedding_type":
            c.embedding_type = {"sinusoidal": 0, "fourier": 1}[cfg.embedding_type]
        elif name == "edge_product":
            ep = cfg.edge_product
            if ep == "f32" and harness_enabled() and os.environ.get("DDMI_EDGE_PRODUCT"):
                ep = os.environ["DDMI_EDGE_PRODUCT"]
            if ep not in EDGE_PRODUCTS:
                raise DdmiError(f"edge_product: unknown route '{ep}' (f32 | bf16x4)")
            c.edge_product = EDGE_PRODUCTS[ep]
        elif name == "exec":
            c.exec = exec_options_from_env(getattr(cfg, "exec_options", None))
        else:
            setattr(c, name, getattr(cfg, name))
    return c


_DECLS = {
    "ddmi_create": (C.c_int, [C.POINTER(Config), C.c_int, C.POINTER(C.c_void_p)]),
    "ddmi_destroy": (None, [C.c_void_p]),
    "ddmi_last_error": (C.c_char_p, []),
    "ddmi_set_weight": (C.c_int, [C.c_void_p, C.c_char_p, C.c_void_p, C.POINTER(C.c_int64), C.c_int]),
    "ddmi_commit_weights": (C.c_int, [C.c_void_p]),
    "ddmi_num_weights": (C.c_int, [C.c_void_p]),
    "ddmi_weight_spec": (C.c_int, [C.c_void_p, C.c_int, C.POINTER(C.c_char_p), C.POINTER(C.c_int64), C.POINTER(C.c_int)]),
    "ddmi_set_table": (C.c_int, [C.c_void_p, C.c_int, C.c_void_p, C.c_int64]),
    "ddmi_set_time_frequencies": (C.c_int, [C.c_void_p, C.c_void_p, C.c_int64]),
    "ddmi_set_complex": (C.c_int, [C.c_void_p, C.POINTER(Complex), C.c_void_p]),
    "ddmi_forward": (C.c_int, [C.c_void_p] + [C.c_void_p] * 7 + [C.c_void_p]),
    "ddmi_confidence": (C.c_int, [C.c_void_p] + [C.c_void_p] * 6 + [C.c_void_p]),
    "ddmi_sidechain_pred": (C.c_int, [C.c_void_p, C.c_void_p, C.c_void_p]),
    "ddmi_set_crop_cutoff": (C.c_int, [C.c_void_p, C.c_float]),
    "ddmi_modify_conformer": (C.c_int, [C.c_void_p] + [C.c_void_p] * 4 + [C.c_void_p]),
    "ddmi_sample": (C.c_int, [C.c_void_p, C.c_void_p, C.POINTER(SampleCfg), C.c_void_p]),
    "ddmi_perturb": (C.c_int, [C.c_void_p, C.c_void_p, C.c_void_p, C.c_void_p, C.POINTER(SampleCfg), C.c_int, C.c_void_p]),
    "ddmi_debug_shape": (C.c_int, [C.c_void_p, C.c_char_p, C.POINTER(C.c_int64), C.POINTER(C.c_int), C.POINTER(C.c_int)]),
    "ddmi_debug_read": (C.c_int, [C.c_void_p, C.c_char_p, C.c_void_p, C.c_size_t, C.c_void_p]),
    "ddmi_wigner_3j": (C.c_int, [C.c_int, C.c_int, C.c_int, C.c_void_p]),
# ... 44 lines not shown
```

include/ddmi.h:

```cpp
#ifndef DDMI_H
#define DDMI_H

#include <stddef.h>
#include <stdint.h>

#ifdef __cplusplus
extern "C" {
#endif

typedef struct ddmi_model ddmi_model;
typedef void* ddmi_stream;

enum ddmi_status {
  DDMI_OK = 0,
  DDMI_ERR_ARG = -1,
  DDMI_ERR_STATE = -2,
  DDMI_ERR_HIP = -3,
  DDMI_ERR_KEY = -4,
  DDMI_ERR_CAPACITY = -5
};

typedef struct ddmi_exec_options {
  int32_t streams;
  int32_t dense_rows;
  int32_t shared_tiles;
  int32_t packed_granules;
  int32_t merged_granule;
  int32_t pre_reduce;
  int32_t hidden_mm;
  int32_t fc1_batch;
  int32_t tile_split;
  int32_t tile_split_small;
  int32_t hidden_grid;
  int32_t tp_apply;
  int32_t debug;
  int32_t tile_per_pose;
  int32_t layer_overlap;
  int32_t grouped;
  int32_t grouped_split;
  int32_t vn_build;
  int32_t node_update;
  int32_t tile_split_last;
  int32_t tile_split_rule;
  int32_t group_order;
  int32_t list_caps;
  int32_t time_terms;
} ddmi_exec_options;

typedef struct ddmi_config {
  uint32_t struct_size;
  int32_t ns, nv, num_conv_layers, num_prot_emb_layers, sh_lmax;
  int32_t sigma_embed_dim, distance_embed_dim, cross_distance_embed_dim, in_lig_edge_features;
  int32_t lm_embedding_dim;
  float lig_max_radius, rec_max_radius, cross_max_distance, center_max_distance;
  int32_t dynamic_max_cross, use_second_order_repr, reduce_pseudoscalars, differentiate_convolutions;
  int32_t embed_also_ligand, batch_norm, smooth_edges, odd_parity, no_torsion, scale_by_sigma;
  int32_t fixed_center_conv;
  float embedding_scale;
  float tr_sigma_min, tr_sigma_max, rot_sigma_min, rot_sigma_max, tor_sigma_min, tor_sigma_max;
  int32_t all_atoms;
  int32_t confidence_mode, num_confidence_outputs;
  int32_t old_model;
  int32_t atom_confidence, atom_num_confidence_outputs, affinity_prediction;
  int32_t embedding_type;
  int32_t tp_weights_layers;
  int32_t sidechain_pred;
  int32_t depthwise_convolution;
  int32_t edge_product;
  ddmi_exec_options exec;
} ddmi_config;

typedef struct ddmi_complex {
  int32_t num_graphs, n_lig, n_rec, n_bond_edges, n_rec_edges, n_tor;
  const int32_t* lig_ptr;
  const int32_t* rec_ptr;
  const int32_t* lig_x;
  const int32_t* bond_index;
  const float* bond_attr;
  const uint8_t* edge_mask;
  const float* rec_x;
  const float* rec_pos;
  const int32_t* rec_edge_index;
  const uint8_t* mask_rotate;
  int32_t n_atom, n_atom_edges, n_atom_rec_edges;
  const int32_t* atom_ptr;
  const int32_t* atom_x;
  const float* atom_pos;
  const int32_t* atom_edge_index;
  const int32_t* atom_rec_edge_index;
} ddmi_complex;

typedef struct ddmi_sample_cfg {
  int32_t inference_steps;
  const double* tr_schedule;
  const double* rot_schedule;
  const double* tor_schedule;
  int32_t ode, no_random, no_final_step_noise;
  double temp_sampling[3], temp_psi[3], temp_sigma_data[3];
  uint64_t seed;
  const int64_t* sample_ids;
  const float* z_tr;
  const float* z_rot;
  const float* z_tor;
  int32_t use_crop;
  double crop_beyond;
} ddmi_sample_cfg;

int ddmi_create(const ddmi_config* cfg, int device, ddmi_model** out);
void ddmi_destroy(ddmi_model* m);
const char* ddmi_last_error(void);

int ddmi_set_weight(ddmi_model* m, const char* key, const float* host_data, const int64_t* shape, int ndim);
int ddmi_commit_weights(ddmi_model* m);
int ddmi_num_weights(ddmi_model* m);
int ddmi_weight_spec(ddmi_model* m, int i, const char** key, int64_t shape[4], int* ndim);

int ddmi_set_table(ddmi_model* m, int kind, const double* host_data, int64_t n);
int ddmi_set_time_frequencies(ddmi_model* m, const float* host_freq, int64_t n);

int ddmi_set_complex(ddmi_model* m, const ddmi_complex* c, ddmi_stream stream);

int ddmi_forward(ddmi_model* m, const float* lig_pos, const float* t_tr, const float* t_rot, const float* t_tor,
                 float* tr_out, float* rot_out, float* tor_out, ddmi_stream stream);

int ddmi_sidechain_pred(ddmi_model* m, float* out, ddmi_stream stream);

int ddmi_confidence(ddmi_model* m, const float* lig_pos, const float* t_tr, const float* t_rot, const float* t_tor,
                    float* conf_out, float* atom_conf_out, ddmi_stream stream);

// ... 23 lines not shown
```

Before: 155.2.

## Share first-layer receptor-receptor messages across identical receptor copies in batch

```diff
diff --git a/diffdock_amd/csrc/api.cpp b/diffdock_amd/csrc/api.cpp
--- a/diffdock_amd/csrc/api.cpp
+++ b/diffdock_amd/csrc/api.cpp
@@ -41,6 +41,7 @@
       in(x.tile_split_small, 8, "tile_split_small"); in(x.hidden_grid, 1 << 20, "hidden_grid"); in(x.tp_apply, 3, "tp_apply");
       in(x.tile_per_pose, 1, "tile_per_pose"); in(x.layer_overlap, 2, "layer_overlap");
       in(x.grouped, 2, "grouped"); in(x.grouped_split, 8, "grouped_split"); in(x.vn_build, 1, "vn_build"); in(x.node_update, 3, "node_update"); in(x.tile_split_last, 8, "tile_split_last"); in(x.tile_split_rule, 2, "tile_split_rule"); in(x.group_order, 3, "group_order"); in(x.list_caps, 1, "list_caps"); in(x.time_terms, 1, "time_terms");
+      in(x.rec_share, 1, "rec_share");
       h->m.two_streams = x.streams == 0;
       h->m.fused_dense = x.dense_rows == 0 ? 1 : x.dense_rows == 1 ? 0 : 2;
       h->m.fused_shared = x.shared_tiles == 0 ? 1 : x.shared_tiles == 1 ? 0 : 2;
@@ -66,6 +67,7 @@
       h->m.group_order = x.group_order;
       h->m.tight_caps = x.list_caps == 1;
       h->m.time_terms_fused = x.time_terms == 1;
+      h->m.rec_share = x.rec_share;
       {
         int cus = 0;
         if (hipDeviceGetAttribute(&cus, hipDeviceAttributeMultiprocessorCount, device) == hipSuccess && cus >= 16) h->m.n_cus = cus;
diff --git a/diffdock_amd/csrc/complex.cpp b/diffdock_amd/csrc/complex.cpp
--- a/diffdock_amd/csrc/complex.cpp
+++ b/diffdock_amd/csrc/complex.cpp
@@ -12,6 +12,8 @@
   int B = 0, nL = 0, nR = 0, N = 0, Eb = 0, Err = 0, nT = 0;
   int maxNl = 0, maxNr = 0, Ell_cap = 0, Elr_cap = 0, tor_cap = 32, Et = 0, lig_cap = 33;
   bool uniform = false; int Nl_one = 0, R_one = 0;
+  bool rec_copies = false; int Rc_one = 0, Erc_one = 0;
+  ReduceGroup* rg_all_share = nullptr;
   std::vector<int> lig_ptr_h, rec_ptr_h;
   int *lig_batch, *rec_batch, *lig_ptr, *rec_ptr, *lig_x;
   int *bond_src, *bond_dst, *bond_grank, *bond_trank, *bg, *bt; float* bond_attr;
@@ -39,10 +41,11 @@
                  float* rows = nullptr;
                  int* tile_hdr = nullptr; unsigned char* live = nullptr;
                  int* nvn_pad = nullptr;
+                 int graphs = 0;
                  const int *built_goff = nullptr, *built_tgt = nullptr, *built_tslot = nullptr, *built_arow = nullptr;
                  const float *built_nvec = nullptr, *built_ew = nullptr; float built_sgn = 0.f; int built_tbase = -1; long epoch = -1; };
   bool prered = false;
-  VnSet vn[9];
+  VnSet vn[10];
   int nA = 0, maxNa = 0, Eaa = 0, Ear = 0, Ela_cap = 0;
   int *atom_batch = nullptr, *atom_ptr = nullptr, *atom_x = nullptr;
   float* atom_pos = nullptr;
@@ -162,14 +165,18 @@
   vr.vcap = vs.vcap; vr.rows = vs.rows; vr.vn_ne = vs.ne;
   return vr;
 }
-static const char vn_type[9] = {'R', 'R', 'L', 'L', 'A', 'A', 'A', 'L', 'R'};
+static const char vn_type[10] = {'R', 'R', 'L', 'L', 'A', 'A', 'A', 'L', 'R', 'R'};
 static void ensure_vn_all(Model& m, const std::vector<RunGroup>& groups, hipStream_t gs) {
   Cx& c = *m.cx;
   VnListsArgs LA;
   VnRowsArgs rows[VN_GROUPS_MAX];
+  const RunGroup* built[VN_GROUPS_MAX];
   const RunGroup* prered_g = nullptr;
   for (auto& g : groups) {
     if (vn_fresh(c, g) || g.gcount <= 0) continue;
+    bool queued = false;
+    for (int i = 0; i < LA.n; ++i) queued = queued || built[i]->vn == g.vn;
+    if (queued) continue;
     DDMI_REQUIRE(LA.n < VN_GROUPS_MAX, DDMI_ERR_CAPACITY, "more edge groups than virtual-node list slots");
     Cx::VnSet& vs = c.vn[g.vn];
     VnListArgs& a = LA.g[LA.n];
@@ -178,15 +185,14 @@
       const bool lig = vn_type[g.vn] == 'L', atom = vn_type[g.vn] == 'A';
       a.node_batch = lig ? c.lig_batch : atom ? c.atom_batch : c.rec_batch;
       a.graph_ptr = lig ? c.lig_ptr : atom ? c.atom_ptr : c.rec_ptr;
-      a.n_graphs = c.B; a.nvn_pad = vs.nvn_pad;
+      a.n_graphs = vs.graphs; a.nvn_pad = vs.nvn_pad;
     }
     rows[LA.n] = vn_rows_args(m, g);
     if (g.vn == 0 && c.prered) {
       prered_g = &g;
       if (m.cfg.sh_lmax <= 1) { rows[LA.n].tile_hdr = vs.tile_hdr; rows[LA.n].live = vs.live; }
     }
-    ++LA.n;
-    vn_mark_built(c, g);
+    built[LA.n++] = &g;
   }
   if (LA.n == 0) return;
   PhaseTimer t(m, "vn_build", gs);
@@ -195,6 +201,7 @@
     Cx::VnSet& vs = c.vn[0];
     launch_vn_tiles(vs.nvn_pad ? vs.nvn_pad : vs.voff + prered_g->gcount, vs.vcap, vs.rows, vs.ne, vs.tile_hdr, vs.live, gs);
   }
+  for (int i = 0; i < LA.n; ++i) vn_mark_built(c, *built[i]);
 }
 static void ensure_vn(Model& m, const RunGroup& g, hipStream_t gs) {
   Cx& c = *m.cx;
@@ -207,7 +214,7 @@
     const bool lig = vn_type[g.vn] == 'L', atom = vn_type[g.vn] == 'A';
     pp.node_batch = lig ? c.lig_batch : atom ? c.atom_batch : c.rec_batch;
     pp.graph_ptr = lig ? c.lig_ptr : atom ? c.atom_ptr : c.rec_ptr;
-    pp.n_graphs = c.B; pp.nvn_pad = vs.nvn_pad;
+    pp.n_graphs = vs.graphs; pp.nvn_pad = vs.nvn_pad;
   }
   launch_vn_build(g.goff, g.gcount, vs.cnt, vs.voff, vs.node, vs.e0, vr, gs, vs.nvn_pad ? &pp : nullptr);
   if (g.vn == 0 && c.prered) launch_vn_tiles(vs.nvn_pad ? vs.nvn_pad : vs.voff + g.gcount, vs.vcap, vs.rows, vs.ne, vs.tile_hdr, vs.live, gs);
@@ -446,6 +453,7 @@
                        L.has_bn ? L.bn_scale : nullptr, L.has_bn ? L.bn_bias : nullptr, L.residual ? 1 : 0, Xin, Xout, XS, s);
       return;
     }
+    DDMI_REQUIRE(rg_dev != c.rg_all_share, DDMI_ERR_STATE, "k_node_update does not fold message rows onto graph 0 (ReduceGroup::tmod)");
     PhaseTimer t(m, "k_reduce_bn", s);
     NodeUpdateArgs a{};
     a.groups = rg_dev; a.n_groups = n_rg; a.nbase = nbase; a.ncount = ncount; a.D_in = L.D_in; a.D_out = L.D_out;
@@ -731,6 +739,20 @@
     rr_tlist[rr_tslot[e]] = e;
     rr_gnode[e] = rr_dst[k];
   }
+  bool copies = c.B > 1 && !cfg.all_atoms && !cfg.old_model && c.Err > 0 && c.Err % c.B == 0;
+  const int R1 = c.rec_ptr_h[1], E1 = copies ? c.Err / c.B : 0;
+  for (int b = 0; b < c.B && copies; ++b) copies = c.rec_ptr_h[b + 1] - c.rec_ptr_h[b] == R1;
+  for (int k = 0; k < c.Err && copies; ++k) {
+    const int q = k / E1, k0 = k - q * E1;
+    copies = rr_src[k] == rr_src[k0] + q * R1 && rr_dst[k] == rr_dst[k0] + q * R1 && rr_src[k0] < R1 && rr_dst[k0] < R1;
+  }
+  int* rec_differ = nullptr;
+  if (copies) {
+    c.Rc_one = R1; c.Erc_one = E1;
+    rec_differ = dalloc<int>(m, nullptr, {1});
+    DDMI_CHECK_HIP(hipMemsetAsync(rec_differ, 0, sizeof(int), s));
+    launch_rows_differ(cc.rec_x, 1 + m.lm, cc.rec_pos, 3, R1, c.B, rec_differ, s);
+  }
   if (cfg.all_atoms) {
     c.atom_batch = dup(m, "atom_batch", atom_batch); c.atom_ptr = dup(m, nullptr, atom_ptr_h);
     c.atom_x = dalloc<int>(m, nullptr, {c.nA * 4});
@@ -844,13 +866,13 @@
   {
     int HKq = 0;
     for (auto* L : all_layers) HKq = std::max(HKq, L->HKq);
-    const int ecap_v[9] = {c.Elr_cap, c.Err, c.Ell_cap, c.Elr_cap, c.Ela_cap, c.Ear, c.Eaa, c.Ela_cap, c.Ear};
-    const int gn_v[9] = {nR, nR, nL, nL, c.nA, c.nA, c.nA, nL, nR};
-    const bool lig_v[9] = {false, false, true, true, false, false, false, true, false};
-    const char* names[9] = {"vn_off_cross", "vn_off_rr", "vn_off_ll", "vn_off_rl", "vn_off_la", "vn_off_ra", "vn_off_aa",
-                            "vn_off_al", "vn_off_ar"};
-    long tight[9];
-    for (int i = 0; i < 9; ++i) tight[i] = -1;
+    const int ecap_v[10] = {c.Elr_cap, c.Err, c.Ell_cap, c.Elr_cap, c.Ela_cap, c.Ear, c.Eaa, c.Ela_cap, c.Ear, E1};
+    const int gn_v[10] = {nR, nR, nL, nL, c.nA, c.nA, c.nA, nL, nR, R1};
+    const bool lig_v[10] = {false, false, true, true, false, false, false, true, false, false};
+    const char* names[10] = {"vn_off_cross", "vn_off_rr", "vn_off_ll", "vn_off_rl", "vn_off_la", "vn_off_ra", "vn_off_aa",
+                             "vn_off_al", "vn_off_ar", "vn_off_rr0"};
+    long tight[10];
+    for (int i = 0; i < 10; ++i) tight[i] = -1;
     auto vn_of = [](long deg) { return (deg + 31) / 32; };
     auto exact = [&](const std::vector<int>& off) { long n = 0; for (size_t d = 0; d + 1 < off.size(); ++d) n += vn_of(off[d + 1] - off[d]); return n; };
     tight[0] = tight[3] = 0;
@@ -860,6 +882,7 @@
       tight[3] += nl * vn_of(nr);
     }
     tight[1] = exact(goff);
+    if (copies) tight[9] = exact(std::vector<int>(goff.begin(), goff.begin() + R1 + 1));
     tight[2] = 0;
     for (int d = 0; d < nL; ++d) tight[2] += vn_of((long)c.lig_cap + bg[d]);
     if (cfg.all_atoms) {
@@ -872,15 +895,17 @@
       tight[5] = exact(h_ra.goff); tight[6] = exact(h_aa.goff); tight[8] = exact(h_ar.goff);
     }
     int vmax = 0, vmax_b = 0;
-    for (int i = 0; i < (cfg.all_atoms ? 9 : 4); ++i) {
+    for (int i = 0; i < 10; ++i) {
+      if (i < 9 ? i >= (cfg.all_atoms ? 9 : 4) : !copies) continue;
       Cx::VnSet& vs = c.vn[i];
+      vs.graphs = i == 9 ? 1 : B;
       vs.vcap = gn_v[i] + ecap_v[i] / 32 + 2;
       if (m.tight_caps && tight[i] >= 0) vs.vcap = (int)std::min<long>(vs.vcap, tight[i] + 2);
       if (m.tile_per_pose) {
-        vs.vcap += 16 * B;
+        vs.vcap += 16 * vs.graphs;
         vs.nvn_pad = dalloc<int>(m, i == 0 ? "vn_count_cross" : nullptr, {1}, true);
       }
-      vs.cnt = dalloc<int>(m, nullptr, {gn_v[i] + 1}); vs.voff = dalloc<int>(m, names[i], {gn_v[i] + 1});
+      vs.cnt = dalloc<int>(m, nullptr, {gn_v[i] + 1}); vs.voff = dalloc<int>(m, names[i], {gn_v[i] + 1}, i == 9);
       vs.node = dalloc<int>(m, nullptr, {vs.vcap}); vs.e0 = dalloc<int>(m, nullptr, {vs.vcap});
       const int shd = (cfg.sh_lmax + 1) * (cfg.sh_lmax + 1);
       vs.ne = dalloc<int>(m, i == 0 ? "vn_ne_cross" : nullptr, {round_up(vs.vcap, 16)});
@@ -908,6 +933,11 @@
                                    {c.rr_toff, c.msg[2], nL, nR}, {c.offs_r, c.msg[3], nL, nR}};
     rg[1].live = c.prered ? c.vn[0].live : nullptr;
     c.rg_all = m.cpool.upload(rg);
+    if (copies) {
+      std::vector<ReduceGroup> rs = rg;
+      rs[2].tmod = R1;
+      c.rg_all_share = m.cpool.upload(rs);
+    }
     std::vector<ReduceGroup> rl(rg.begin(), rg.begin() + 2);
     c.rg_lig = m.cpool.upload(rl);
     std::vector<ReduceGroup> r0(rg.begin(), rg.begin() + 1);
@@ -1056,6 +1086,11 @@
       DDMI_CHECK_HIP(hipMemcpyAsync(c.rec_node_base, xin, (size_t)nR * XS * 4, hipMemcpyDeviceToDevice, s));
   }
   DDMI_CHECK_HIP(hipStreamSynchronize(s));
+  if (rec_differ) {
+    int differ = 1;
+    DDMI_CHECK_HIP(hipMemcpy(&differ, rec_differ, sizeof(int), hipMemcpyDeviceToHost));
+    c.rec_copies = differ == 0;
+  }
   m.has_complex = true;
 }
 
@@ -1413,10 +1448,14 @@
       }
       if (gb.n) launch_gemm_batch(gb, s);
     }
+    const bool rec_share = m.rec_share == 0 && m.uniform_t && c.rec_copies && !crop && !overlapped && !nu && m.grouped != 2 && Lc >= 2;
+    RunGroup g_rr0 = g_rr;
+    g_rr0.gcount = g_rr0.tcount = c.Rc_one; g_rr0.ea_rows = c.Erc_one; g_rr0.vn = 9; g_rr0.static_topo = true;
     if (overlapped) run_conv_layers_overlapped(m, g_ll, g_lr, g_rr, g_rl, crop ? c.rg_all_crop : c.rg_all, xi, s);
     else
     for (int l = 0; l < Lc; ++l, ++xi) {
-      RunGroup rr = g_rr;
+      const bool share = rec_share && l == 0;
+      RunGroup rr = share ? g_rr0 : g_rr;
       if (nu && l < Lc - 1) rr.rb_ready = c.rb_l[l];
       const std::vector<RunGroup> full = {g_ll, g_lr, rr, g_rl}, ligs = {g_ll, g_lr};
       std::vector<RunGroup> next;
@@ -1426,7 +1465,8 @@
       const int pq = !nu ? 0 : l == 0 ? 1 : 2;
       const ConvW* Ln = next.empty() ? nullptr : &m.conv_layers[l + 1];
       if (l < Lc - 1)
-        run_conv(m, m.conv_layers[l], full, crop ? c.rg_all_crop : c.rg_all, 4, c.X[xi], c.X[xi + 1], 0, c.N, s, pq, Ln, Ln ? &next : nullptr);
+        run_conv(m, m.conv_layers[l], full, share ? c.rg_all_share : crop ? c.rg_all_crop : c.rg_all, 4, c.X[xi], c.X[xi + 1], 0, c.N, s, pq, Ln,
+                 Ln ? &next : nullptr);
       else run_conv(m, m.conv_layers[l], ligs, c.rg_lig, 2, c.X[xi], c.X[xi + 1], 0, cfg.sidechain_pred ? c.N : nL, s, pq);
     }
   }
@@ -1575,7 +1615,14 @@
     float* tk = times_once ? c.s_t + (size_t)k * 3 * B : c.s_t;
     if (!times_once) launch_fill_times(tk, B, (float)t_tr, (float)t_rot, (float)t_tor, s);
     m.crop_cutoff = sc.use_crop ? s_tr * 3.0 + sc.crop_beyond : 0.0;
-    forward(m, lig_pos, tk, tk + B, tk + 2 * B, c.s_tr, c.s_rot, torsion ? c.s_tor : nullptr, s);
+    {
+      struct UniformT {
+        Model& m;
+        explicit UniformT(Model& mm) : m(mm) { m.uniform_t = true; }
+        ~UniformT() { m.uniform_t = false; }
+      } uniform_t{m};
+      forward(m, lig_pos, tk, tk + B, tk + 2 * B, c.s_tr, c.s_rot, torsion ? c.s_tor : nullptr, s);
+    }
     perturb_step(m, c.s_tr, c.s_rot, torsion ? c.s_tor : nullptr, sc, k, ids_dev, s);
 #ifdef DDMI_PROFILING
     static const bool freeze = getenv("DDMI_FREEZE_POSE") != nullptr;
diff --git a/diffdock_amd/csrc/k_conv.hip b/diffdock_amd/csrc/k_conv.hip
--- a/diffdock_amd/csrc/k_conv.hip
+++ b/diffdock_amd/csrc/k_conv.hip
@@ -310,8 +310,9 @@
   int cnt = 0;
   for (int g = 0; g < n_groups; ++g) {
     const ReduceGroup G = groups[g];
-    const int sl = s - G.tbase;
+    int sl = s - G.tbase;
     if (sl < 0 || sl >= G.tcount) continue;
+    if (G.tmod > 0) sl %= G.tmod;
     const int b = G.toff[sl], e = G.toff[sl + 1];
     cnt += e - b;
     if (G.live) {
diff --git a/diffdock_amd/csrc/k_graph.hip b/diffdock_amd/csrc/k_graph.hip
--- a/diffdock_amd/csrc/k_graph.hip
+++ b/diffdock_amd/csrc/k_graph.hip
@@ -283,6 +283,26 @@
   DDMI_CHECK_HIP(hipGetLastError());
 }
 
+__global__ void k_rows_differ(const float* __restrict__ a, int lda, const float* __restrict__ b, int ldb, int n_one, long total,
+                              int* __restrict__ differ) {
+  const int ld = lda + ldb;
+  for (long i = (long)blockIdx.x * blockDim.x + threadIdx.x; i < total; i += (long)gridDim.x * blockDim.x) {
+    const long row = n_one + i / ld;
+    const int col = (int)(i % ld);
+    const long row0 = row % n_one;
+    const unsigned* p = reinterpret_cast<const unsigned*>(col < lda ? a : b);
+    const int w = col < lda ? lda : ldb, c = col < lda ? col : col - lda;
+    if (p[row * w + c] != p[row0 * w + c]) *differ = 1;
+  }
+}
+void launch_rows_differ(const float* a, int lda, const float* b, int ldb, int n_one, int copies, int* differ, hipStream_t s) {
+  const long total = (long)n_one * (copies - 1) * (lda + ldb);
+  if (total <= 0) return;
+  const int blocks = cdiv(total, 256);
+  hipLaunchKernelGGL(k_rows_differ, dim3(blocks < 2048 ? blocks : 2048), dim3(256), 0, s, a, lda, b, ldb, n_one, total, differ);
+  DDMI_CHECK_HIP(hipGetLastError());
+}
+
 __global__ void k_rr_filter_count(const int* __restrict__ keep, const int* __restrict__ goff, const int* __restrict__ tgt,
                                   const int* __restrict__ toff, const int* __restrict__ tlist,
                                   const int* __restrict__ gnode, int nL, int nR, int* __restrict__ cnt_g,
diff --git a/diffdock_amd/csrc/kernels.h b/diffdock_amd/csrc/kernels.h
--- a/diffdock_amd/csrc/kernels.h
+++ b/diffdock_amd/csrc/kernels.h
@@ -134,7 +134,7 @@
 static_assert(sizeof(FusedGroupedArgs) <= 3072, "kernel arguments of k_conv_grouped (4 KB limit)");
 void launch_conv_grouped(const FusedGroupedArgs& G, hipStream_t s);
 
-struct ReduceGroup { const int* toff; const float* msg; int tbase, tcount; const unsigned char* live = nullptr; };
+struct ReduceGroup { const int* toff; const float* msg; int tbase, tcount; const unsigned char* live = nullptr; int tmod = 0; };
 void launch_reduce_bn(const ReduceGroup* groups_dev, int n_groups, int nbase, int ncount, int D_in, int D_out,
                       const float* bn_mean, const float* bn_scale, const float* bn_bias, int residual,
                       const float* X_in, float* X_out, int out_stride, hipStream_t s);
@@ -166,6 +166,7 @@
                         const int* keep, int* pairrank, int* cnt_l, int* cnt_r, hipStream_t s);
 void launch_crop_mask(const float* lpos, const float* rpos, const int* rbatch, const int* lptr, int nR, float cut2, int* keep,
                       hipStream_t s);
+void launch_rows_differ(const float* a, int lda, const float* b, int ldb, int n_one, int copies, int* differ, hipStream_t s);
 void launch_rr_filter(const int* keep, const int* goff, const int* tgt, const int* arow, const int* toff, const int* tlist,
                       const int* gnode, int nL, int nR, int* cnt_g, int* cnt_t, int* goff2, int* toff2, int* tslot_tmp,
                       int* tgt2, int* tslot2, int* arow2, hipStream_t s);
diff --git a/diffdock_amd/csrc/model.h b/diffdock_amd/csrc/model.h
--- a/diffdock_amd/csrc/model.h
+++ b/diffdock_amd/csrc/model.h
@@ -117,6 +117,8 @@
   bool node_update = false;
   bool vn_merge = true;
   bool tile_per_pose = false;
+  int rec_share = 0;
+  bool uniform_t = false;
   double crop_cutoff = 0.0;
   DevicePool cpool;
   struct Cx;
diff --git a/diffdock_amd/lib.py b/diffdock_amd/lib.py
--- a/diffdock_amd/lib.py
+++ b/diffdock_amd/lib.py
@@ -20,7 +20,8 @@
 class ExecOptions(C.Structure):
     _fields_ = [(n, C.c_int32) for n in ("streams", "dense_rows", "shared_tiles", "packed_granules", "merged_granule", "pre_reduce",
                                          "hidden_mm", "fc1_batch", "tile_split", "tile_split_small", "hidden_grid", "tp_apply",
-                                         "debug", "tile_per_pose", "layer_overlap", "grouped", "grouped_split", "vn_build", "node_update", "tile_split_last", "tile_split_rule", "group_order", "list_caps", "time_terms")]
+                                         "debug", "tile_per_pose", "layer_overlap", "grouped", "grouped_split", "vn_build", "node_update", "tile_split_last", "tile_split_rule", "group_order", "list_caps", "time_terms",
+                                         "rec_share")]
 
 
 def harness_enabled() -> bool:
@@ -79,6 +80,7 @@
             raise DdmiError("DDMI_GROUPED: 0 / 1 (per-group launches) or 2 (grouped)")
         x.grouped = e("DDMI_GROUPED")
     if e("DDMI_GROUPED_YS") is not None: x.grouped_split = max(0, min(8, e("DDMI_GROUPED_YS")))
+    if e("DDMI_REC_SHARE") is not None: x.rec_share = 0 if e("DDMI_REC_SHARE") != 0 else 1
     return x
 
 
diff --git a/include/ddmi.h b/include/ddmi.h
--- a/include/ddmi.h
+++ b/include/ddmi.h
@@ -45,6 +45,7 @@
   int32_t group_order;
   int32_t list_caps;
   int32_t time_terms;
+  int32_t rec_share;
 } ddmi_exec_options;
 
 typedef struct ddmi_config {
```

After: 158.2 (median of 6 runs). +1.9%, better.
